# artpixls/ART

Hardware: AMD Instinct MI355X
Metric: megapixels/sec end-to-end (AMaZE+FTblockDN+tone), 45 MP Bayer (higher is better)
Workload: dtype f32; 1 GPU; AMaZE + getImage/matrix + ImProcFunctions::denoise (chroma noise-curve map, FTblockDN wavelet shrinkage luma 40 / chroma 15 / gamma 1.7 + DCT detail recovery 50) + exposure 0.3 EV + tone curve STD, 8192x5464 Bayer RGGB fp32, 1 frame per GPU per step (BASELINE configs[2]); frame=8192x5464, lanes_per_gpu=1, parallelism=frame-per-gpu x1, completion_records=1, completion_via=single process

## Files before the change

### art_amd/csrc/artgpu_api.hip

```cpp
#include <hip/hip_runtime.h>
#include <dlfcn.h>
#include <cmath>
#include <cstdio>
#include <cstdarg>
#include <cstring>
#include <new>
#include <string>
#include <thread>
#include <vector>
#include <algorithm>

#include "../../include/artgpu.h"
#include "kernels.h"
#include "dehaze.h"
#include "textureboost.h"
#include "colorcorrection.h"
#include "smoothing.h"
#include "masks.h"
#include "sharpen.h"

using namespace artgpu;

struct artgpu_ctx {
    int device = 0;
    hipStream_t stream = nullptr;
    hipStream_t aux = nullptr;
    hipEvent_t aux_ev[2] = {nullptr, nullptr};
    hipStream_t dn_stream[1] = {nullptr};
    hipEvent_t dn_ev[2] = {nullptr, nullptr};
    const float *gam_tab = nullptr; float gam_key[6] = {};
    struct Shared {
        int opt_sharpen_fused = 1;
        int opt_lut_lds = 1;
        int opt_dn_streams = 0;
        int opt_dn_fused = 1;
        int opt_dn_detail_plain = 0;
        int opt_dn_debug_stall = -1;
        long opt_dn_wait_ms = 0;
        int opt_io_direct = -1;
        int opt_amaze_path = 0;
        int opt_amaze_split = 0;
        long opt_amaze_zero_mask = 0x81f0;
        int opt_amaze_zero_frame = 16;
        int opt_amaze_poison = -1;
        int opt_roctx = 0;
        int opt_amaze_overlap = 1;
        int opt_amaze_grid = 0;
        int opt_rcd_rows = 8;
        int curve_tail_kind = ARTGPU_CURVE_TAIL_HOST;
        double curve_tail_y = 1.0;
        ParamCurve curve_tail_pc = {};
        artgpu_progress_fn progress_fn = nullptr;
        void *progress_user = nullptr;
        const artgpu_mask_params *pipe_lc = nullptr, *pipe_tb = nullptr;
        int pipe_nlc = 0, pipe_ntb = 0;
        const artgpu_color_correction_region *pipe_cc = nullptr;
        const artgpu_mask_params *pipe_cc_masks = nullptr;
        int pipe_ncc = 0;
        const artgpu_smoothing_region *pipe_sm = nullptr;
        const artgpu_mask_params *pipe_sm_masks = nullptr;
        int pipe_nsm = 0;
    } shared;
    float *sh_host = nullptr;
    hipEvent_t sh_ev = nullptr;
    struct PipeMasks { std::vector<artgpu_mask_params> m; std::vector<std::vector<double>> curves; std::vector<artgpu_plane> areas; } pipe_lc_own, pipe_tb_own;
    template <typename Region> struct PipeRegions { std::vector<Region> regs; std::vector<artgpu_plane> planes; PipeMasks masks; };
    PipeRegions<artgpu_color_correction_region> pipe_cc_own;
    PipeRegions<artgpu_smoothing_region> pipe_sm_own;
    std::string err;
    int *fs_diag = nullptr;
    long long batch_px = 0;
    int dn_form = -1, dn_form_streak = 0;
    float *arena = nullptr;
    size_t arena_bytes = 0;
    static constexpr int NSTAGE = 8;
    float *stage[NSTAGE] = {};
    size_t stage_bytes[NSTAGE] = {};
    static constexpr int NPOOL = 96;
    float *pool[NPOOL] = {};
    size_t pool_bytes[NPOOL] = {};
    std::vector<artgpu_ctx *> lanes;
    int batch_lanes = 1;
    int frames_in_flight = 1;
    bool owns_stream = false;
    hipStream_t io_up = nullptr, io_down = nullptr;
    hipEvent_t io_ev[8] = {};
    int *io_host = nullptr;
    int io_host_cap = 0;
    int cu_reserve = 0;
    float *bbox = nullptr;
    size_t bbox_bytes = 0;
    float *amz_lists = nullptr;
    size_t amz_lists_bytes = 0;
    int amz_w = 0, amz_h = 0, amz_nstream = 0, amz_narena = 0, amz_mode = -1;
    int num_cus = 0;
    hipStream_t amz_side = nullptr;
    hipEvent_t amz_ev[2] = {nullptr, nullptr};
    int *rcd_counter = nullptr;
    float *lut = nullptr;
    size_t lut_bytes = 0;
    std::vector<float> lut_host;
    std::vector<float> ncurve_host;
    char *tab_ring = nullptr;
    size_t tab_ring_bytes = 0, tab_ring_off = 0;
    bool tab_ring_busy = false;
    hipEvent_t tab_ev = nullptr;
    std::vector<float> rgbcurve_host[3];
    bool timing = false;
    hipEvent_t ev[3] = {nullptr, nullptr, nullptr};
    artgpu_timings last = {0.f, 0.f, 0.f};
};

namespace {

int fail(artgpu_ctx *ctx, int code, const char *fmt, ...)
{
    char buf[512];
    va_list ap;
    va_start(ap, fmt);
    vsnprintf(buf, sizeof buf, fmt, ap);
    va_end(ap);
    if (ctx) {
        ctx->err = buf;
        if (code == ARTGPU_EHIP && ctx->fs_diag && (unsigned)ctx->fs_diag[0] == 0xF5D1A600u) {
            char more[192];
            snprintf(more, sizeof more, " [shrink_blur_kernel: band %d strip %d gave up waiting for the strip above to hand down block %d (its counter: %d)]",
                     ctx->fs_diag[1], ctx->fs_diag[2], ctx->fs_diag[3], ctx->fs_diag[4]);
            ctx->err += more;
            ctx->fs_diag[0] = 0;
        }
    }
    return code;
}

#define HIPCHK(ctx, call)                                                                        \
    do {                                                                                         \
        hipError_t e_ = (call);                                                                  \
        if (e_ != hipSuccess)                                                                    \
            return fail(ctx, ARTGPU_EHIP, "%s failed: %s (%s:%d)", #call, hipGetErrorString(e_), __FILE__, __LINE__); \
    } while (0)

struct SideStreamJoin {
    hipStream_t side = nullptr;
    void arm(hipStream_t s) { side = s; }
    void disarm() { side = nullptr; }
    ~SideStreamJoin() { if (side) (void)hipStreamSynchronize(side); }
};

int ensure(artgpu_ctx *ctx, float **buf, size_t *cur, size_t need)
{
    if (*cur >= need) return ARTGPU_OK;
    if (*buf) { HIPCHK(ctx, hipFree(*buf)); *buf = nullptr; *cur = 0; }
    hipError_t e = hipMalloc(reinterpret_cast<void **>(buf), need);
    if (e != hipSuccess) {
        *buf = nullptr;
        return fail(ctx, ARTGPU_ENOMEM, "hipMalloc(%zu bytes) failed: %s", need, hipGetErrorString(e));
    }
    *cur = need;
    return ARTGPU_OK;
}

int h2d_table(artgpu_ctx *ctx, void *dst, const void *src, size_t bytes)
{
    const size_t need = (bytes + 255) & ~(size_t)255;
    if (need > ctx->tab_ring_bytes) {
        if (ctx->tab_ring) {
            if (ctx->tab_ring_busy) HIPCHK(ctx, hipEventSynchronize(ctx->tab_ev));
            HIPCHK(ctx, hipHostFree(ctx->tab_ring));
            ctx->tab_ring = nullptr; ctx->tab_ring_bytes = 0; ctx->tab_ring_busy = false;
        }
        const size_t cap = need * 2 > ((size_t)8 << 20) ? need * 2 : ((size_t)8 << 20);
        if (hipHostMalloc(reinterpret_cast<void **>(&ctx->tab_ring), cap, hipHostMallocDefault) != hipSuccess) {
            ctx->tab_ring = nullptr;
            return fail(ctx, ARTGPU_ENOMEM, "pinned staging ring for look-up tables (%zu bytes)", cap);
        }
        ctx->tab_ring_bytes = cap; ctx->tab_ring_off = 0;
        if (!ctx->tab_ev) HIPCHK(ctx, hipEventCreateWithFlags(&ctx->tab_ev, hipEventDisableTiming));
    }
    if (ctx->tab_ring_off + need > ctx->tab_ring_bytes) {
        if (ctx->tab_ring_busy) HIPCHK(ctx, hipEventSynchronize(ctx->tab_ev));
        ctx->tab_ring_busy = false;
        ctx->tab_ring_off = 0;
    }
    char *slot = ctx->tab_ring + ctx->tab_ring_off;
    std::memcpy(slot, src, bytes);
    HIPCHK(ctx, hipMemcpyAsync(dst, slot, bytes, hipMemcpyHostToDevice, ctx->stream));
    HIPCHK(ctx, hipEventRecord(ctx->tab_ev, ctx->stream));
    ctx->tab_ring_busy = true;
    ctx->tab_ring_off += need;
    return ARTGPU_OK;
}

bool plane_ok(const artgpu_plane *p)
{
    return p && p->p && p->w > 0 && p->h > 0 && p->row_stride_bytes >= (int64_t)p->w * 4 && (p->row_stride_bytes % 4) == 0;
}

struct DevImage {
    const float *raw; size_t raw_stride;
    float *r, *g, *b; size_t out_stride;
    bool staged;
};

int bind_images(artgpu_ctx *ctx, const artgpu_plane *raw, artgpu_rgb *out, DevImage *d)
{
    const int W = raw->w, H = raw->h;
    const artgpu_plane *op[3] = {&out->r, &out->g, &out->b};
    for (int k = 0; k < 3; ++k) {
        if (!plane_ok(op[k]) || op[k]->w != W || op[k]->h != H) return fail(ctx, ARTGPU_EINVAL, "output plane %d: bad pointer/size/stride", k);
        if ((op[k]->on_device != 0) != (out->r.on_device != 0) || op[k]->row_stride_bytes != out->r.row_stride_bytes)
            return fail(ctx, ARTGPU_EINVAL, "output planes must share residency and row stride");
    }
    d->staged = false;
    if (raw->on_device) {
        d->raw = raw->p;
        d->raw_stride = (size_t)(raw->row_stride_bytes / 4);
    } else {
        int rc = ensure(ctx, &ctx->stage[0], &ctx->stage_bytes[0], (size_t)W * H * 4);
        if (rc) return rc;
        HIPCHK(ctx, hipMemcpy2DAsync(ctx->stage[0], (size_t)W * 4, raw->p, (size_t)raw->row_stride_bytes, (size_t)W * 4, H, hipMemcpyHostToDevice, ctx->stream));
        d->raw = ctx->stage[0];
        d->raw_stride = W;
    }
    if (out->r.on_device) {
// ... 80 lines not shown
    d->staged = true;
    return ARTGPU_OK;
}

int unbind_rgb(artgpu_ctx *ctx, artgpu_rgb *img, const DevRGB *d)
{
    if (!d->staged) return ARTGPU_OK;
    artgpu_plane *pl[3] = {&img->r, &img->g, &img->b};
    const size_t rowb = (size_t)d->w * 4;
    for (int k = 0; k < 3; ++k)
        HIPCHK(ctx, hipMemcpy2DAsync(pl[k]->p, (size_t)pl[k]->row_stride_bytes, d->p[k], rowb, rowb, d->h, hipMemcpyDeviceToHost, ctx->stream));
    HIPCHK(ctx, hipStreamSynchronize(ctx->stream));
    return ARTGPU_OK;
}

#ifndef ARTGPU_MAX_TILE_WG
#define ARTGPU_MAX_TILE_WG 8192
#endif
constexpr int MAX_TILE_WORKGROUPS = ARTGPU_MAX_TILE_WG;

}

extern "C" {

const char *artgpu_version(void) { return "artgpu 0.1 (gfx950)"; }

int artgpu_create(int hip_device, artgpu_ctx **out)
{
    if (!out) return ARTGPU_EINVAL;
    *out = nullptr;
    int n = 0;
    if (hipGetDeviceCount(&n) != hipSuccess || n <= 0 || hip_device < 0 || hip_device >= n) return ARTGPU_EHIP;
    artgpu_ctx *ctx = new (std::nothrow) artgpu_ctx;
    if (!ctx) return ARTGPU_ENOMEM;
    ctx->device = hip_device;
    if (hipSetDevice(hip_device) != hipSuccess) { delete ctx; return ARTGPU_EHIP; }
    for (int k = 0; k < 3; ++k)
        if (hipEventCreate(&ctx->ev[k]) != hipSuccess) {
            for (int j = 0; j < k; ++j) (void)hipEventDestroy(ctx->ev[j]);
            delete ctx;
            return ARTGPU_EHIP;
        }
    *out = ctx;
    return ARTGPU_OK;
}

int artgpu_destroy(artgpu_ctx *ctx)
{
    if (!ctx) return ARTGPU_EINVAL;
    (void)hipSetDevice(ctx->device);
    (void)hipStreamSynchronize(ctx->stream);
    if (ctx->arena) (void)hipFree(ctx->arena);
    for (int k = 0; k < artgpu_ctx::NSTAGE; ++k)
        if (ctx->stage[k]) (void)hipFree(ctx->stage[k]);
    if (ctx->lut) (void)hipFree(ctx->lut);
    if (ctx->tab_ring) (void)hipHostFree(ctx->tab_ring);
    if (ctx->fs_diag) (void)hipHostFree(ctx->fs_diag);
    if (ctx->sh_host) (void)hipHostFree(ctx->sh_host);
    if (ctx->sh_ev) (void)hipEventDestroy(ctx->sh_ev);
    if (ctx->tab_ev) (void)hipEventDestroy(ctx->tab_ev);
    if (ctx->bbox) (void)hipFree(ctx->bbox);
    if (ctx->amz_lists) (void)hipFree(ctx->amz_lists);
    if (ctx->rcd_counter) (void)hipFree(ctx->rcd_counter);
    for (int k = 0; k < artgpu_ctx::NPOOL; ++k)
        if (ctx->pool[k]) (void)hipFree(ctx->pool[k]);
    for (int k = 0; k < 3; ++k)
        if (ctx->ev[k]) (void)hipEventDestroy(ctx->ev[k]);
    for (artgpu_ctx *l : ctx->lanes) (void)artgpu_destroy(l);
    ctx->lanes.clear();
    if (ctx->io_up) { (void)hipStreamSynchronize(ctx->io_up); (void)hipStreamDestroy(ctx->io_up); }
    if (ctx->io_down) { (void)hipStreamSynchronize(ctx->io_down); (void)hipStreamDestroy(ctx->io_down); }
    for (int k = 0; k < 8; ++k)
        if (ctx->io_ev[k]) (void)hipEventDestroy(ctx->io_ev[k]);
    if (ctx->io_host) (void)hipHostFree(ctx->io_host);
    if (ctx->owns_stream && ctx->stream) (void)hipStreamDestroy(ctx->stream);
    for (int k = 0; k < 2; ++k)
        if (ctx->aux_ev[k]) (void)hipEventDestroy(ctx->aux_ev[k]);
    if (ctx->aux) { (void)hipStreamSynchronize(ctx->aux); (void)hipStreamDestroy(ctx->aux); }
    for (int k = 0; k < 2; ++k)
        if (ctx->dn_ev[k]) (void)hipEventDestroy(ctx->dn_ev[k]);
    if (ctx->dn_stream[0]) { (void)hipStreamSynchronize(ctx->dn_stream[0]); (void)hipStreamDestroy(ctx->dn_stream[0]); }
    for (int k = 0; k < 2; ++k)
        if (ctx->amz_ev[k]) (void)hipEventDestroy(ctx->amz_ev[k]);
    if (ctx->amz_side) { (void)hipStreamSynchronize(ctx->amz_side); (void)hipStreamDestroy(ctx->amz_side); }
    delete ctx;
    return ARTGPU_OK;
}

const char *artgpu_last_error(const artgpu_ctx *ctx) { return ctx ? ctx->err.c_str() : "null context"; }

int artgpu_set_stream(artgpu_ctx *ctx, void *hip_stream)
{
    if (!ctx) return ARTGPU_EINVAL;
    hipStream_t next = static_cast<hipStream_t>(hip_stream);
    if (next == ctx->stream) return ARTGPU_OK;
    HIPCHK(ctx, hipSetDevice(ctx->device));
    hipEvent_t ev = nullptr;
    if (hipEventCreateWithFlags(&ev, hipEventDisableTiming) == hipSuccess) {
        if (hipEventRecord(ev, ctx->stream) == hipSuccess) (void)hipStreamWaitEvent(next, ev, 0);
        (void)hipEventDestroy(ev);
    }
    (void)hipGetLastError();
    ctx->stream = next;
    return ARTGPU_OK;
}

static int check_async_faults(artgpu_ctx *ctx)
{
    if (ctx->fs_diag && (unsigned)ctx->fs_diag[0] == 0xF5D1A600u) return fail(ctx, ARTGPU_EHIP, "a kernel gave up a bounded wait: the results of the calls since the last synchronisation are invalid");
    return ARTGPU_OK;
}

int artgpu_synchronize(artgpu_ctx *ctx)
{
    if (!ctx) return ARTGPU_EINVAL;
    HIPCHK(ctx, hipSetDevice(ctx->device));
    HIPCHK(ctx, hipStreamSynchronize(ctx->stream));
    return check_async_faults(ctx);
}

int artgpu_set_curve_tail(artgpu_ctx *ctx, int kind, double y_last)
{
    if (!ctx) return ARTGPU_EINVAL;
    if (kind < ARTGPU_CURVE_TAIL_LUT || kind > ARTGPU_CURVE_TAIL_HOST) return fail(ctx, ARTGPU_EINVAL, "set_curve_tail: kind %d (a parametric curve: artgpu_set_curve_tail_parametric)", kind);
    ctx->shared.curve_tail_kind = kind;
    ctx->shared.curve_tail_y = y_last;
    return ARTGPU_OK;
}

int artgpu_set_curve_tail_parametric(artgpu_ctx *ctx, const double *p, int np)
{
    if (!ctx) return ARTGPU_EINVAL;
    if (!p || (np != 8 && np != 9)) return fail(ctx, ARTGPU_EINVAL, "set_curve_tail_parametric: 8 or 9 parameters (p[0] = DCT_Parametric)");
    if (p[4] == 0.0 && p[5] == 0.0 && p[6] == 0.0 && p[7] == 0.0) return fail(ctx, ARTGPU_EINVAL, "set_curve_tail_parametric: an identity curve has no Curve object (ARTGPU_CURVE_TAIL_LUT)");
    pc_init(ctx->shared.curve_tail_pc, p, np);
    ctx->shared.curve_tail_kind = ARTGPU_CURVE_TAIL_PARAMETRIC;
    return ARTGPU_OK;
}

int artgpu_get_option(artgpu_ctx *ctx, const char *name, long *value)
{
    if (!ctx || !name || !value) return ARTGPU_EINVAL;
    const std::string n(name);
    if (n.rfind("amaze_counter", 0) == 0 && n.size() == 14 && n[13] >= '0' && n[13] <= '7') {
        if (!ctx->amz_lists || ctx->amz_nstream <= 0) { *value = 0; return ARTGPU_OK; }
        HIPCHK(ctx, hipSetDevice(ctx->device));
        HIPCHK(ctx, hipStreamSynchronize(ctx->stream));
        const size_t nfixed = (((size_t)ctx->amz_nstream + (1 + ctx->amz_narena) + (1 + ctx->amz_narena + ctx->amz_nstream) + 3) / 4) * 4;
        int v = 0;
        HIPCHK(ctx, hipMemcpy(&v, reinterpret_cast<int *>(ctx->amz_lists) + nfixed + 4 + 2 * (size_t)ctx->amz_nstream + (n[13] - '0'), sizeof(int), hipMemcpyDeviceToHost));
        *value = v;
        return ARTGPU_OK;
    }
    return fail(ctx, ARTGPU_EINVAL, "get_option: unknown option '%s'", name);
}

int artgpu_set_option(artgpu_ctx *ctx, const char *name, long value)
{
    if (!ctx || !name) return ARTGPU_EINVAL;
    const std::string n(name);
    if (n == "amaze_path") { if (value < 0 || value > 1) return fail(ctx, ARTGPU_EINVAL, "amaze_path: 0 or 1"); ctx->shared.opt_amaze_path = (int)value; }
    else if (n == "amaze_split") ctx->shared.opt_amaze_split = value != 0;
    else if (n == "amaze_overlap") ctx->shared.opt_amaze_overlap = value != 0;
    else if (n == "amaze_grid") { if (value < 0) return fail(ctx, ARTGPU_EINVAL, "amaze_grid: >= 0"); ctx->shared.opt_amaze_grid = (int)value; }
    else if (n == "amaze_zero_mask") ctx->shared.opt_amaze_zero_mask = value;
    else if (n == "amaze_zero_frame") ctx->shared.opt_amaze_zero_frame = (int)value;
    else if (n == "amaze_poison") ctx->shared.opt_amaze_poison = (int)value;
    else if (n == "roctx") ctx->shared.opt_roctx = value != 0;
    else if (n == "dn_streams") ctx->shared.opt_dn_streams = value != 0;
    else if (n == "dn_fused") ctx->shared.opt_dn_fused = (int)value;
    else if (n == "dn_detail_plain") { if (value < 0 || value > 3) return fail(ctx, ARTGPU_EINVAL, "dn_detail_plain: 0 .. 3"); ctx->shared.opt_dn_detail_plain = (int)value; }
    else if (n == "dn_debug_stall") ctx->shared.opt_dn_debug_stall = (int)value;
    else if (n == "dn_wait_ms") ctx->shared.opt_dn_wait_ms = value < 0 ? 0 : value;
    else if (n == "lut_lds") ctx->shared.opt_lut_lds = value != 0;
    else if (n == "sharpen_fused") ctx->shared.opt_sharpen_fused = value != 0;
    else if (n == "cu_reserve") { if (value < 0 || value > 4096) return fail(ctx, ARTGPU_EINVAL, "cu_reserve: 0 .. 4096"); ctx->cu_reserve = (int)value; }
    else if (n == "io_direct") { if (value < -1 || value > 4096) return fail(ctx, ARTGPU_EINVAL, "io_direct: -1 (automatic), 0 .. 4096 workgroups"); ctx->shared.opt_io_direct = (int)value; }
    else if (n == "rcd_rows") { if (value != 4 && value != 8) return fail(ctx, ARTGPU_EINVAL, "rcd_rows: 4 or 8"); ctx->shared.opt_rcd_rows = (int)value; }
    else return fail(ctx, ARTGPU_EINVAL, "set_option: unknown option '%s'", name);
    return ARTGPU_OK;
}

int artgpu_set_progress_callback(artgpu_ctx *ctx, artgpu_progress_fn fn, void *user)
{
    if (!ctx) return ARTGPU_EINVAL;
    ctx->shared.progress_fn = fn;
    ctx->shared.progress_user = user;
    return ARTGPU_OK;
}

int artgpu_enable_timing(artgpu_ctx *ctx, int enable)
{
    if (!ctx) return ARTGPU_EINVAL;
    ctx->timing = enable != 0;
    return ARTGPU_OK;
}

int artgpu_get_timings(const artgpu_ctx *ctx, artgpu_timings *out)
{
    if (!ctx || !out) return ARTGPU_EINVAL;
    *out = ctx->last;
    return ARTGPU_OK;
}

size_t artgpu_scratch_bytes(const artgpu_ctx *ctx)
{
    if (!ctx) return 0;
    size_t s = ctx->arena_bytes;
    for (int k = 0; k < artgpu_ctx::NSTAGE; ++k) s += ctx->stage_bytes[k];
    s += ctx->lut_bytes;
    for (int k = 0; k < artgpu_ctx::NPOOL; ++k) s += ctx->pool_bytes[k];
    return s;
}

int artgpu_trim_scratch(artgpu_ctx *ctx)
{
    if (!ctx) return ARTGPU_EINVAL;
    HIPCHK(ctx, hipSetDevice(ctx->device));
    HIPCHK(ctx, hipStreamSynchronize(ctx->stream));
    if (ctx->aux) HIPCHK(ctx, hipStreamSynchronize(ctx->aux));
    if (ctx->dn_stream[0]) HIPCHK(ctx, hipStreamSynchronize(ctx->dn_stream[0]));
    if (ctx->amz_side) HIPCHK(ctx, hipStreamSynchronize(ctx->amz_side));
    if (ctx->io_up) HIPCHK(ctx, hipStreamSynchronize(ctx->io_up));
    if (ctx->io_down) HIPCHK(ctx, hipStreamSynchronize(ctx->io_down));
    auto drop = [](float **p, size_t *b) { if (*p) (void)hipFree(*p); *p = nullptr; *b = 0; };
    drop(&ctx->arena, &ctx->arena_bytes);
    for (int k = 0; k < artgpu_ctx::NSTAGE; ++k) drop(&ctx->stage[k], &ctx->stage_bytes[k]);
    for (int k = 0; k < artgpu_ctx::NPOOL; ++k) drop(&ctx->pool[k], &ctx->pool_bytes[k]);
    ctx->batch_px = 0;
    ctx->gam_tab = nullptr;
    ctx->ncurve_host.clear();
    for (int k = 0; k < 3; ++k) ctx->rgbcurve_host[k].clear();
    int rc = ARTGPU_OK;
    for (artgpu_ctx *l : ctx->lanes) { const int r = artgpu_trim_scratch(l); if (r && !rc) rc = r; }
    return rc;
}

struct StageScope {
    artgpu_ctx *ctx;
    const char *name;
    bool range;
    typedef int (*push_fn)(const char *);
    typedef int (*pop_fn)();
    static push_fn &push() { static push_fn f = nullptr; return f; }
    static pop_fn &pop() { static pop_fn f = nullptr; return f; }
    StageScope(artgpu_ctx *c, const char *n) : ctx(c), name(n), range(false)
    {
        if (!ctx) return;
        if (ctx->shared.opt_roctx) {
            static bool tried = false;
            if (!tried) {
                tried = true;
                void *h = nullptr;
                for (const char *lib : {"libroctx64.so.4", "libroctx64.so", "/opt/rocm/lib/libroctx64.so"})
                    if ((h = dlopen(lib, RTLD_NOW | RTLD_GLOBAL))) break;
                if (h) {
                    push() = reinterpret_cast<push_fn>(dlsym(h, "roctxRangePushA"));
                    pop() = reinterpret_cast<pop_fn>(dlsym(h, "roctxRangePop"));
                }
            }
            if (push() && pop()) { push()(name); range = true; }
        }
        if (ctx->shared.progress_fn) ctx->shared.progress_fn(ctx->shared.progress_user, name, 0.0);
    }
    ~StageScope()
    {
        if (!ctx) return;
        if (ctx->shared.progress_fn) ctx->shared.progress_fn(ctx->shared.progress_user, name, 1.0);
        if (range) pop()();
    }
};

struct DualReq { double *contrast; int auto_contrast; int second; };
static int vng4_dev(artgpu_ctx *ctx, const float *raw, size_t raw_stride, float *r, float *g, float *b, size_t out_stride, int W, int H, uint32_t filters);
static int dual_blend_dev(artgpu_ctx *ctx, const DevImage &d, int W, int H, uint32_t filters, DualReq *req);
static int demosaic_bayer_impl(artgpu_ctx *ctx, int method, const artgpu_plane *raw, uint32_t filters,
                               double initial_gain, int border, artgpu_rgb *out, DualReq *dual)
{
    StageScope scope_(ctx, "RawImageSource::demosaic (Bayer)");
    if (!ctx) return ARTGPU_EINVAL;
    if (!plane_ok(raw) || !out) return fail(ctx, ARTGPU_EINVAL, "demosaic_bayer: bad raw plane or null output");
    if (method != ARTGPU_BAYER_AMAZE && method != ARTGPU_BAYER_RCD && method != ARTGPU_BAYER_VNG4) return fail(ctx, ARTGPU_EUNSUPPORTED, "demosaic_bayer: method %d is not on the device path", method);
    if (!(initial_gain > 0.0)) return fail(ctx, ARTGPU_EINVAL, "demosaic_bayer: initial_gain must be > 0");
    for (unsigned r = 0; r < 2; ++r)
        for (unsigned c = 0; c < 2; ++c)
            if (((filters >> ((((r << 1) & 14) + (c & 1)) << 1)) & 3) == 3) return fail(ctx, ARTGPU_EUNSUPPORTED, "demosaic_bayer: 4-colour CFA");
    const int W = raw->w, H = raw->h;
    if (W < 64 || H < 64) return fail(ctx, ARTGPU_EUNSUPPORTED, "demosaic_bayer: image %dx%d smaller than 64x64", W, H);
    HIPCHK(ctx, hipSetDevice(ctx->device));

    DevImage d;
    int rc = bind_images(ctx, raw, out, &d);
    if (rc) return rc;
    if (ctx->timing) HIPCHK(ctx, hipEventRecord(ctx->ev[0], ctx->stream));

    int bord = 0;
    if (method == ARTGPU_BAYER_AMAZE) {
        const int nty = (H + 16 + AMAZE_STEP - 1) / AMAZE_STEP, ntx = (W + 16 + AMAZE_STEP - 1) / AMAZE_STEP;
        const int ntiles = nty * ntx;
        const int mode = ctx->shared.opt_amaze_path;
        if (ctx->amz_w != W || ctx->amz_h != H || ctx->amz_mode != mode) {
            std::vector<int> st, ar;
            for (int ty = 0; ty < nty; ++ty)
                for (int tx = 0; tx < ntx; ++tx) {
                    const int top = -16 + ty * AMAZE_STEP, left = -16 + tx * AMAZE_STEP;
                    const int rr1 = std::min(top + AMAZE_TS, H + 16) - top, cc1 = std::min(left + AMAZE_TS, W + 16) - left;
                    if (rr1 <= 32 || cc1 <= 32) continue;
                    const bool wide = cc1 == AMAZE_TS && (left + AMAZE_TS <= W || left + AMAZE_TS == W + 16);
                    const bool rows_ok = rr1 < AMAZE_TS || top + AMAZE_TS <= H || top + AMAZE_TS == H + 16;
                    (mode == 0 && wide && rows_ok ? st : ar).push_back(ty * ntx + tx);
                }
            const size_t nfixed = ((st.size() + (1 + ar.size()) + (1 + ar.size() + st.size()) + 3) / 4) * 4;
            const size_t nints = nfixed + 4 + 2 * st.size() + 8;
            if ((rc = ensure(ctx, &ctx->amz_lists, &ctx->amz_lists_bytes, nints * sizeof(int)))) return rc;
            std::vector<int> hostbuf;
            hostbuf.insert(hostbuf.end(), st.begin(), st.end());
            hostbuf.push_back((int)ar.size());
            hostbuf.insert(hostbuf.end(), ar.begin(), ar.end());
            HIPCHK(ctx, hipMemcpyAsync(ctx->amz_lists, hostbuf.data(), hostbuf.size() * sizeof(int), hipMemcpyHostToDevice, ctx->stream));
            HIPCHK(ctx, hipStreamSynchronize(ctx->stream));
            ctx->amz_w = W; ctx->amz_h = H; ctx->amz_mode = mode;
            ctx->amz_nstream = (int)st.size(); ctx->amz_narena = (int)ar.size();
        }
        int *const d_stream = reinterpret_cast<int *>(ctx->amz_lists);
        int *const d_templ = d_stream + ctx->amz_nstream;
        int *const d_work = d_templ + 1 + ctx->amz_narena;
        const size_t nfixed = (((size_t)ctx->amz_nstream + (1 + ctx->amz_narena) + (1 + ctx->amz_narena + ctx->amz_nstream) + 3) / 4) * 4;
        int *const d_queue = d_stream + nfixed;
        unsigned long long *const d_qwords = reinterpret_cast<unsigned long long *>(d_queue + 4);
        const float clip_pt = (float)(1.0 / initial_gain);
        const float clip_pt8 = (float)(0.8 / initial_gain);
        const bool split = mode == 1 && ctx->shared.opt_amaze_split;
        const bool early = ctx->amz_nstream > 0 && ctx->amz_narena > 0 && ctx->shared.opt_amaze_overlap;
        const int nlist_max = ctx->amz_narena + ctx->amz_nstream;
        const int cap = split ? MAX_TILE_WORKGROUPS : 768;
        const int grid = split ? std::min(ntiles, cap) : std::max(1, std::min(nlist_max, cap));
        rc = ensure(ctx, &ctx->arena, &ctx->arena_bytes, (size_t)grid * AMAZE_ARENA_FLOATS * sizeof(float));
        if (rc) return rc;
        if ((rc = ensure(ctx, &ctx->bbox, &ctx->bbox_bytes, (size_t)grid * 4 * sizeof(int)))) return rc;
        AmazeArgs a;
        a.raw = d.raw; a.raw_stride = d.raw_stride;
        a.red = d.r; a.green = d.g; a.blue = d.b; a.out_stride = d.out_stride;
        a.arena = ctx->arena;
        a.W = W; a.H = H; a.ntx = ntx; a.ntiles = ntiles;
        a.filters = filters;
        a.clip_pt = clip_pt;
        a.clip_pt8 = clip_pt8;
        a.bbox = reinterpret_cast<int *>(ctx->bbox);
        a.zero_mask = (unsigned)ctx->shared.opt_amaze_zero_mask;
        a.zero_frame = ctx->shared.opt_amaze_zero_frame;
        a.split = split ? 1 : 0;
        a.queue_words = d_qwords;
        a.queue_counters = reinterpret_cast<int *>(d_qwords + ctx->amz_nstream);
        if (ctx->shared.opt_amaze_poison >= 0)
            HIPCHK(ctx, hipMemsetAsync(ctx->arena, ctx->shared.opt_amaze_poison, (size_t)grid * AMAZE_ARENA_FLOATS * sizeof(float), ctx->stream));
        HIPCHK(ctx, hipMemsetAsync(d_queue, 0, (4 + 2 * (size_t)ctx->amz_nstream + 8) * sizeof(int), ctx->stream));
        SideStreamJoin amz_join;
        if (early) {
            HIPCHK(ctx, hipMemsetAsync(d_work, 0, sizeof(int), ctx->stream));
            if (!ctx->amz_side) {
                HIPCHK(ctx, hipStreamCreateWithFlags(&ctx->amz_side, hipStreamNonBlocking));
                for (int k = 0; k < 2; ++k) HIPCHK(ctx, hipEventCreateWithFlags(&ctx->amz_ev[k], hipEventDisableTiming));
            }
            HIPCHK(ctx, hipEventRecord(ctx->amz_ev[0], ctx->stream));
            HIPCHK(ctx, hipStreamWaitEvent(ctx->amz_side, ctx->amz_ev[0], 0));
            amz_join.arm(ctx->amz_side);
            a.tile_list = d_templ + 1; a.tile_count = d_templ;
            a.queue_hdr = nullptr;
            HIPCHK(ctx, launch_amaze(a, std::min(ctx->amz_narena, cap), ctx->stream));
        } else {
            HIPCHK(ctx, hipMemcpyAsync(d_work, d_templ, (size_t)(1 + ctx->amz_narena) * sizeof(int), hipMemcpyDeviceToDevice, ctx->stream));
        }
        if (ctx->amz_nstream > 0) {
            AmazeStreamArgs sa;
            sa.raw = d.raw; sa.raw_stride = d.raw_stride;
            sa.red = d.r; sa.green = d.g; sa.blue = d.b; sa.out_stride = d.out_stride;
            sa.W = W; sa.H = H; sa.ntx = ntx;
            sa.filters = filters;
            sa.clip_pt = clip_pt; sa.clip_pt8 = clip_pt8;
            const unsigned f00 = (filters >> 0) & 3, f01 = (filters >> 2) & 3;
            sa.g00 = (int)(f00 & 1);
            sa.ey = f00 == 1 ? (f01 == 0 ? 0 : 1) : (f00 == 0 ? 0 : 1);
            sa.tiles = d_stream; sa.ntiles = ctx->amz_nstream;
// ... 224 lines not shown
namespace {
int wavelet_skip(int level) { return level <= 1 ? 1 : 1 << (level - 1); }
}

extern "C" {

int artgpu_wavelet_decompose(artgpu_ctx *ctx, const artgpu_plane *src, int maxlvl, artgpu_wavelet **out)
{
    if (!ctx) return ARTGPU_EINVAL;
    if (!plane_ok(src) || !out || maxlvl < 1 || maxlvl > 9) return fail(ctx, ARTGPU_EINVAL, "wavelet_decompose: bad arguments");
    *out = nullptr;
    const int w = src->w, h = src->h, w2 = (w + 1) / 2, h2 = (h + 1) / 2;
    if ((w2 < h2 ? w2 : h2) < 2 * wavelet_skip(maxlvl - 1) || w < 8 || h < 8)
        return fail(ctx, ARTGPU_EUNSUPPORTED, "wavelet_decompose: %dx%d too small for %d levels", w, h, maxlvl);
    HIPCHK(ctx, hipSetDevice(ctx->device));
    const float *dsrc = src->p;
    size_t sstride = (size_t)(src->row_stride_bytes / 4);
    if (!src->on_device) {
        int rc = ensure(ctx, &ctx->stage[0], &ctx->stage_bytes[0], (size_t)w * h * 4);
        if (rc) return rc;
        HIPCHK(ctx, hipMemcpy2DAsync(ctx->stage[0], (size_t)w * 4, src->p, (size_t)src->row_stride_bytes, (size_t)w * 4, h, hipMemcpyHostToDevice, ctx->stream));
        dsrc = ctx->stage[0];
        sstride = w;
    }
    artgpu_wavelet *wv = new (std::nothrow) artgpu_wavelet;
    if (!wv) return fail(ctx, ARTGPU_ENOMEM, "wavelet_decompose: out of host memory");
    wv->w = w; wv->h = h; wv->w2 = w2; wv->h2 = h2; wv->nlevels = maxlvl; wv->n = (size_t)w2 * h2;
    hipError_t e = hipMalloc(reinterpret_cast<void **>(&wv->bands), (size_t)maxlvl * 3 * wv->n * sizeof(float));
    if (e == hipSuccess) e = hipMalloc(reinterpret_cast<void **>(&wv->lowpass[0]), wv->n * sizeof(float));
    if (e == hipSuccess) e = hipMalloc(reinterpret_cast<void **>(&wv->lowpass[1]), wv->n * sizeof(float));
    if (e != hipSuccess) {
        artgpu_wavelet_free(ctx, wv);
        return fail(ctx, ARTGPU_ENOMEM, "wavelet_decompose: hipMalloc failed: %s", hipGetErrorString(e));
    }
    WaveArgs a = {};
    a.w = w; a.h = h; a.w2 = w2; a.h2 = h2;
    for (int l = 0; l < maxlvl; ++l) {
        a.b1 = wv->band(l, 1); a.b2 = wv->band(l, 2); a.b3 = wv->band(l, 3);
        hipError_t le;
        if (l == 0) {
            a.src = dsrc; a.src_stride = sstride; a.lo = wv->lowpass[0];
            wv->cur = 0;
            le = launch_wavelet_analysis0(a, ctx->stream);
        } else {
            a.src = wv->lowpass[wv->cur]; a.lo = wv->lowpass[wv->cur ^ 1]; a.skip = wavelet_skip(l);
            le = launch_wavelet_haar_analysis(a, ctx->stream);
            wv->cur ^= 1;
        }
        if (le != hipSuccess) {
            artgpu_wavelet_free(ctx, wv);
            return fail(ctx, ARTGPU_EHIP, "wavelet_decompose: launch failed: %s", hipGetErrorString(le));
        }
    }
    if (!src->on_device) {
        const hipError_t se = hipStreamSynchronize(ctx->stream);
        if (se != hipSuccess) {
            artgpu_wavelet_free(ctx, wv);
            return fail(ctx, ARTGPU_EHIP, "wavelet_decompose: %s", hipGetErrorString(se));
        }
    }
    *out = wv;
    return ARTGPU_OK;
}

int artgpu_wavelet_info(const artgpu_wavelet *wv, int32_t *w2, int32_t *h2, int32_t *nlevels)
{
    if (!wv) return ARTGPU_EINVAL;
    if (w2) *w2 = wv->w2;
    if (h2) *h2 = wv->h2;
    if (nlevels) *nlevels = wv->nlevels;
    return ARTGPU_OK;
}

int artgpu_wavelet_get_band(artgpu_ctx *ctx, const artgpu_wavelet *wv, int level, int dir, float *dst, int on_device)
{
    if (!ctx) return ARTGPU_EINVAL;
    if (!wv || !dst || dir < 0 || dir > 3 || (dir > 0 && (level < 0 || level >= wv->nlevels))) return fail(ctx, ARTGPU_EINVAL, "wavelet_get_band: bad arguments");
    HIPCHK(ctx, hipSetDevice(ctx->device));
    const float *p = dir == 0 ? wv->lowpass[wv->cur] : wv->band(level, dir);
    HIPCHK(ctx, hipMemcpyAsync(dst, p, wv->n * sizeof(float), on_device ? hipMemcpyDeviceToDevice : hipMemcpyDeviceToHost, ctx->stream));
    if (!on_device) HIPCHK(ctx, hipStreamSynchronize(ctx->stream));
    return ARTGPU_OK;
}

int artgpu_wavelet_set_band(artgpu_ctx *ctx, artgpu_wavelet *wv, int level, int dir, const float *src, int on_device)
{
    if (!ctx) return ARTGPU_EINVAL;
    if (!wv || !src || dir < 0 || dir > 3 || (dir > 0 && (level < 0 || level >= wv->nlevels))) return fail(ctx, ARTGPU_EINVAL, "wavelet_set_band: bad arguments");
    HIPCHK(ctx, hipSetDevice(ctx->device));
    float *p = dir == 0 ? wv->lowpass[wv->cur] : wv->band(level, dir);
    HIPCHK(ctx, hipMemcpyAsync(p, src, wv->n * sizeof(float), on_device ? hipMemcpyDeviceToDevice : hipMemcpyHostToDevice, ctx->stream));
    if (!on_device) HIPCHK(ctx, hipStreamSynchronize(ctx->stream));
    return ARTGPU_OK;
}

int artgpu_wavelet_reconstruct(artgpu_ctx *ctx, artgpu_wavelet *wv, artgpu_plane *dst, float blend)
{
    if (!ctx) return ARTGPU_EINVAL;
    if (!wv || !plane_ok(dst) || dst->w != wv->w || dst->h != wv->h) return fail(ctx, ARTGPU_EINVAL, "wavelet_reconstruct: bad arguments");
    HIPCHK(ctx, hipSetDevice(ctx->device));
    float *ddst = dst->p;
    size_t dstride = (size_t)(dst->row_stride_bytes / 4);
    if (!dst->on_device) {
        int rc = ensure(ctx, &ctx->stage[0], &ctx->stage_bytes[0], (size_t)wv->w * wv->h * 4);
        if (rc) return rc;
        HIPCHK(ctx, hipMemcpy2DAsync(ctx->stage[0], (size_t)wv->w * 4, dst->p, (size_t)dst->row_stride_bytes, (size_t)wv->w * 4, wv->h, hipMemcpyHostToDevice, ctx->stream));
        ddst = ctx->stage[0];
        dstride = wv->w;
    }
    WaveArgs a = {};
    a.w = wv->w; a.h = wv->h; a.w2 = wv->w2; a.h2 = wv->h2; a.blend = blend;
    for (int l = wv->nlevels - 1; l > 0; --l) {
        a.src = wv->lowpass[wv->cur]; a.lo = wv->lowpass[wv->cur ^ 1];
        a.b1 = wv->band(l, 1); a.b2 = wv->band(l, 2); a.b3 = wv->band(l, 3); a.skip = wavelet_skip(l);
        HIPCHK(ctx, launch_wavelet_haar_synthesis(a, ctx->stream));
        wv->cur ^= 1;
    }
    a.src = wv->lowpass[wv->cur];
    a.b1 = wv->band(0, 1); a.b2 = wv->band(0, 2); a.b3 = wv->band(0, 3);
    a.dst = ddst; a.dst_stride = dstride;
    HIPCHK(ctx, launch_wavelet_synthesis0(a, ctx->stream));
    if (!dst->on_device) {
        HIPCHK(ctx, hipMemcpy2DAsync(dst->p, (size_t)dst->row_stride_bytes, ddst, (size_t)wv->w * 4, (size_t)wv->w * 4, wv->h, hipMemcpyDeviceToHost, ctx->stream));
        HIPCHK(ctx, hipStreamSynchronize(ctx->stream));
    }
    return ARTGPU_OK;
}

int artgpu_wavelet_free(artgpu_ctx *ctx, artgpu_wavelet *wv)
{
    if (!wv) return ARTGPU_EINVAL;
    if (ctx) { (void)hipSetDevice(ctx->device); (void)hipStreamSynchronize(ctx->stream); }
    if (wv->bands) (void)hipFree(wv->bands);
    if (wv->lowpass[0]) (void)hipFree(wv->lowpass[0]);
    if (wv->lowpass[1]) (void)hipFree(wv->lowpass[1]);
    delete wv;
    return ARTGPU_OK;
}

}

namespace {

enum { P_L = 0, P_A, P_B, P_LBANDS, P_LLOW0, P_LLOW1, P_CBANDS, P_CLOW0, P_CLOW1, P_SF, P_TMP, P_HISTO, P_MAD, P_GAM, P_CCALC, P_LIN, P_BLOCKS, P_DTAB, P_CCMAP, P_CACHEF, P_PQ, P_XCBRT, P_GAUSS64, P_DMASK, P_LABTABS, P_PIPE_R, P_PIPE_G, P_PIPE_B, P_DNINFO, P_BATCH, P_DCTTAB, P_CBANDS2, P_CLOW0_2, P_CLOW1_2, P_SF_A, P_SF_B, P_HISTO_A, P_HISTO_B, P_RGBCURVES, P_FUSED, P_LBANDS2,
       P_IO_IN0, P_IO_IN1, P_IO_CFA, P_IO_IMG0, P_IO_IMG1, P_IO_IMG2, P_IO_IMG3, P_IO_IMG4, P_IO_IMG5, P_IO_OUT0, P_IO_OUT1, P_IO_FLAGS,
       P_CA_HALF, P_CA_BLK, P_CA_GUARD, P_CA_RAW,
       P_LC_BANDS, P_LC_LOW0, P_LC_LOW1, P_LC_NEW, P_LC_STATS, P_LC_MASK, P_LC_L,
       P_DH_STATE, P_DH_THUMB, P_DH_LOW, P_DH_TMP, P_DH_T, P_DH_DARK,
       P_SH_PLANES, P_SH_BYTES, P_SH_STATE,
       P_TB_PLANES, P_TB_LOW, P_TB_TMP, P_TB_STATE, P_TB_MASK, P_TB_Y,
       P_MK_WORK, P_MK_TAB, P_MK_CTHR, P_MK_AREA, P_MK_OUT,
       P_CC_MASK, P_CC_OOR, P_CC_GEN,
       P_SM_PLANES, P_SM_MASK, P_SM_BOX, P_SM_GEN,
       P_NSLOTS };
static_assert(P_NSLOTS <= artgpu_ctx::NPOOL, "grow artgpu_ctx::pool");

struct DevDecomp {
    float *bands, *low[2];
    int cur, nlevels, w, h, w2, h2;
    size_t n;
    float *band(int l, int dir) const { return bands + ((size_t)l * 3 + (dir - 1)) * n; }
};

int decompose_dev(artgpu_ctx *ctx, DevDecomp &d, const float *src, hipStream_t st = nullptr, size_t src_stride = 0)
{
    if (!st) st = ctx->stream;
    WaveArgs a = {};
    a.w = d.w; a.h = d.h; a.w2 = d.w2; a.h2 = d.h2;
    for (int l = 0; l < d.nlevels; ++l) {
        a.b1 = d.band(l, 1); a.b2 = d.band(l, 2); a.b3 = d.band(l, 3);
        if (l == 0) {
            a.src = src; a.src_stride = src_stride ? src_stride : (size_t)d.w; a.lo = d.low[0]; d.cur = 0;
            HIPCHK(ctx, launch_wavelet_analysis0(a, st));
        } else {
            a.src = d.low[d.cur]; a.lo = d.low[d.cur ^ 1]; a.skip = wavelet_skip(l);
            HIPCHK(ctx, launch_wavelet_haar_analysis(a, st));
            d.cur ^= 1;
        }
    }
    return ARTGPU_OK;
}

int reconstruct_dev(artgpu_ctx *ctx, DevDecomp &d, float *dst, hipStream_t st = nullptr)
{
    if (!st) st = ctx->stream;
    WaveArgs a = {};
    a.w = d.w; a.h = d.h; a.w2 = d.w2; a.h2 = d.h2; a.blend = 1.f;
    for (int l = d.nlevels - 1; l > 0; --l) {
        a.src = d.low[d.cur]; a.lo = d.low[d.cur ^ 1];
        a.b1 = d.band(l, 1); a.b2 = d.band(l, 2); a.b3 = d.band(l, 3); a.skip = wavelet_skip(l);
        HIPCHK(ctx, launch_wavelet_haar_synthesis(a, st));
        d.cur ^= 1;
    }
    a.src = d.low[d.cur];
    a.b1 = d.band(0, 1); a.b2 = d.band(0, 2); a.b3 = d.band(0, 3);
    a.dst = dst; a.dst_stride = d.w;
    HIPCHK(ctx, launch_wavelet_synthesis0(a, st));
    return ARTGPU_OK;
}

int pool_get(artgpu_ctx *ctx, int slot, size_t bytes, float **out)
{
    int rc = ensure(ctx, &ctx->pool[slot], &ctx->pool_bytes[slot], bytes);
    *out = ctx->pool[slot];
    return rc;
}

}

extern "C" {

namespace {
int detail_mask_dev(artgpu_ctx *ctx, const float *src, size_t src_stride, float *mask, int W, int H,
                    float scaling, float threshold, float ceiling, float factor, float blur, float *scratch);
}

int artgpu_wavelet_mad(artgpu_ctx *ctx, const artgpu_wavelet *wv, float *mad_sqr)
{
    if (!ctx) return ARTGPU_EINVAL;
    if (!wv || !mad_sqr) return fail(ctx, ARTGPU_EINVAL, "wavelet_mad: null argument");
    if (wv->n > 0x7fffffff) return fail(ctx, ARTGPU_EUNSUPPORTED, "wavelet_mad: band larger than an int holds (MadRgb's datalen is an int)");
    HIPCHK(ctx, hipSetDevice(ctx->device));
    const int nsub = 3 * wv->nlevels;
    float *histo_f, *mad;
    int rc;
    if ((rc = pool_get(ctx, P_HISTO, (size_t)nsub * (65536 + MAD_SCRATCH_INTS_PER_BAND) * 4, &histo_f)) || (rc = pool_get(ctx, P_MAD, 3 * 32 * 4, &mad))) return rc;
    HIPCHK(ctx, launch_mad(wv->bands, wv->n, nsub, reinterpret_cast<int *>(histo_f), mad, ctx->stream));
    HIPCHK(ctx, hipMemcpyAsync(mad_sqr, mad, (size_t)nsub * sizeof(float), hipMemcpyDeviceToHost, ctx->stream));
    HIPCHK(ctx, hipStreamSynchronize(ctx->stream));
    return ARTGPU_OK;
}

}

namespace {

struct DnFusion {
    float pre_scale, post_scale;
    GetImageFuse gi;
    int exp_on;
    float exp_scale, exp_black;
    int tail_on;
    float tail_scale, tail_black;
    int ccalc_nonneg;
};

int const_table_dev(artgpu_ctx *ctx, int slot, size_t nfloats, void (*fill)(float *), const char *what, float **out)
{
    const bool fresh = ctx->pool[slot] == nullptr;
    const int rc = pool_get(ctx, slot, nfloats * 4, out);
    if (rc || !fresh) return rc;
    std::vector<float> host(nfloats);
    fill(host.data());
    hipError_t e = hipMemcpyAsync(*out, host.data(), nfloats * 4, hipMemcpyHostToDevice, ctx->stream);
    if (e == hipSuccess) e = hipStreamSynchronize(ctx->stream);
    if (e != hipSuccess) {
        (void)hipFree(ctx->pool[slot]); ctx->pool[slot] = nullptr; ctx->pool_bytes[slot] = 0;
        *out = nullptr;
        return fail(ctx, ARTGPU_EHIP, "upload of the %s failed: %s", what, hipGetErrorString(e));
    }
    return ARTGPU_OK;
}

void build_lab_tabs(float *host)
{
    build_cachef(host); build_cachefy(host + 65536);
    build_denoise_gamma_tabs(host + 2 * 65536, host + 3 * 65536);
}

int lab_tabs_dev(artgpu_ctx *ctx, float **tabs_out)
{
    return const_table_dev(ctx, P_LABTABS, 4 * 65536, build_lab_tabs, "Lab tables", tabs_out);
}

void build_dct_tabs(float *host)
{
    float *tm_in = host, *tm_out = tm_in + 4096, *ct = tm_out + 4096, *ctt = ct + 4096;
    const float epsilon = 0.001f / (64 * 64);
    const int border = 4;
    for (int i = 0; i < 64; ++i) {
        const float i1 = std::abs((i > 32 ? i - 64 + 1 : i));
        const float vmask = (i1 < border ? (float)0 + (std::sin((M_PI * i1) / (2 * border)) * std::sin((M_PI * i1) / (2 * border))) : 1.0f);
        const float vmask2 = (i1 < 2 * border ? (std::sin((M_PI * i1) / (2 * border)) * std::sin((M_PI * i1) / (2 * border))) : 1.0f);
        for (int j = 0; j < 64; ++j) {
            const float j1 = std::abs((j > 32 ? j - 64 + 1 : j));
            const double sj = std::sin((M_PI * j1) / (2 * border));
            tm_in[i * 64 + j] = (vmask * (j1 < border ? sj * sj : 1.0f)) + epsilon;
            tm_out[i * 64 + j] = (vmask2 * (j1 < 2 * border ? sj * sj : 1.0f)) + epsilon;
            ct[i * 64 + j] = (float)std::cos(M_PI * (j + 0.5) * i / 64.0);
            ctt[j * 64 + i] = ct[i * 64 + j];
        }
    }
}

struct DnPlan {
    int w, h, w2, h2;
    size_t n, n2;
    bool lab_mode, do_detail, useNoiseCCurve;
    float noisevarL;
    bool denoiseLuminance;
    float gam, gamthresh, gamslope, igam, igamthresh, igamslope, gain;
    float realred, realblue, noisevarab_r, noisevarab_b, maxNoiseVarab;
    bool aggressive, autoch;
    int levwav, nsub;
    bool too_small;
    int rad[10], maxrad;
    bool fork;
    bool fused, merged, merged_mad;
    bool two_chroma;
    int detail_plain;
    long long wait_ticks;
    int stall_band, stall_strip;
};

DnPlan dn_plan(int w, int h, const artgpu_denoise_params *p, double scale, double expcomp, uint32_t flags, bool want_resid, bool has_ccalc,
               int opt_dn_streams, int opt_dn_fused, int opt_dn_detail_plain, long opt_dn_wait_ms, int opt_dn_debug_stall)
{
    DnPlan pl = {};
    const int w2 = (w + 1) / 2, h2 = (h + 1) / 2;
    pl.w = w; pl.h = h; pl.w2 = w2; pl.h2 = h2; pl.n = (size_t)w * h; pl.n2 = (size_t)w2 * h2;
    pl.lab_mode = p->color_space == 1;
    pl.do_detail = !(flags & ARTGPU_DN_SKIP_DETAIL_RECOVERY);
    pl.useNoiseCCurve = has_ccalc;
    pl.detail_plain = opt_dn_detail_plain == 1 ? 3 : opt_dn_detail_plain == 2 ? 1 : opt_dn_detail_plain == 3 ? 2 : 0;
    pl.wait_ticks = (long long)opt_dn_wait_ms * 100000LL;
    pl.stall_band = opt_dn_debug_stall < 0 ? -1 : opt_dn_debug_stall >> 16;
    pl.stall_strip = opt_dn_debug_stall < 0 ? -1 : opt_dn_debug_stall & 0xffff;

    const float noiseluma = (float)p->luminance;
    const double nl_t = (noiseluma / 125.0) * (1.0 + noiseluma / 25.0);
    const float noisevarL = (float)(nl_t * nl_t);
    const bool denoiseLuminance = noisevarL > 0.00001f;
    const float gam = (float)p->gamma;
    const float gamthresh = 0.001f;
    const float gamslope = (float)(std::exp(std::log((double)gamthresh) / gam) / gamthresh);
    pl.noisevarL = noisevarL; pl.denoiseLuminance = denoiseLuminance;
    pl.gam = gam; pl.gamthresh = gamthresh; pl.gamslope = gamslope;
    pl.igam = 1.f / gam; pl.igamthresh = gamthresh * gamslope; pl.igamslope = 1.f / gamslope;
    pl.gain = std::pow(2.0f, float(expcomp));
    const float interm_med = (float)p->chrominance / 10.0;
    float intermred = p->chrominance_red_green > 0. ? (p->chrominance_red_green / 10.) : (float)p->chrominance_red_green / 7.0;
    float intermblue = p->chrominance_blue_yellow > 0. ? (p->chrominance_blue_yellow / 10.) : (float)p->chrominance_blue_yellow / 7.0;
    float realred = interm_med + intermred;
    if (realred <= 0.f) realred = 0.001f;
    float realblue = interm_med + intermblue;
    if (realblue <= 0.f) realblue = 0.001f;
    const float noisevarab_r = realred * realred, noisevarab_b = realblue * realblue;
    pl.realred = realred; pl.realblue = realblue; pl.noisevarab_r = noisevarab_r; pl.noisevarab_b = noisevarab_b;
    pl.maxNoiseVarab = noisevarab_b > noisevarab_r ? noisevarab_b : noisevarab_r;
    int levwav = 5;
    const float maxreal = realred > realblue ? realred : realblue;
    if (maxreal < 8.f) levwav = 5; else if (maxreal < 10.f) levwav = 6; else if (maxreal < 15.f) levwav = 7; else levwav = 8;
    const bool aggressive = p->aggressive != 0;
    if (aggressive) levwav += 2;
    if (levwav > 8) levwav = 8;
    { const int t = int(levwav - std::ceil(std::log(scale))); levwav = t > 5 ? t : 5; }
    const int minsizetile = w < h ? w : h;
    int maxlev2 = 8;
    if (minsizetile < 256) maxlev2 = 7;
    if (minsizetile < 128) maxlev2 = 6;
    if (minsizetile < 64) maxlev2 = 5;
    if (minsizetile < 32) maxlev2 = 4;
    if (minsizetile < 16) maxlev2 = 3;
    levwav = levwav < maxlev2 ? levwav : maxlev2;
    const int nsub = 3 * levwav;
    const bool autoch = p->chrominance_method == 1;
    pl.aggressive = aggressive; pl.autoch = autoch; pl.levwav = levwav; pl.nsub = nsub;
    pl.too_small = (w2 < h2 ? w2 : h2) < 2 * wavelet_skip(levwav - 1) || w < 8 || h < 8;
    if (pl.too_small) return pl;

    pl.fork = opt_dn_streams != 0 && pl.do_detail && denoiseLuminance;

    pl.maxrad = 1;
    for (int l = 0; l < levwav; ++l) { const int r = int((l + 2) / scale); pl.rad[l] = r > 1 ? r : 1; pl.maxrad = pl.rad[l] > pl.maxrad ? pl.rad[l] : pl.maxrad; }
    pl.fused = opt_dn_fused != 0 && shrink_blur_supported(w2, h2, pl.rad, 0, nsub);
    pl.merged = pl.fused && opt_dn_fused != 2 && !aggressive && !want_resid && denoiseLuminance && levwav <= 5 &&
                (autoch || (noisevarab_r > 0.001f && noisevarab_b > 0.001f));
    pl.merged_mad = pl.merged && opt_dn_fused != 3;
    pl.two_chroma = pl.fork || pl.merged;
    return pl;
}

struct DnBuffers {
    float *L, *A, *B, *gamlut, *mad, *ccalc_dev;
    float *sfc[3], *tmpc[3], *histo_fc[3];
    DevDecomp Ld, Cdd[2];
    float *fused_scratch, *Lbands2;
};

int pool_drop(artgpu_ctx *ctx, int slot)
{
    if (!ctx->pool[slot]) return ARTGPU_OK;
    HIPCHK(ctx, hipStreamSynchronize(ctx->stream));
    if (ctx->dn_stream[0]) HIPCHK(ctx, hipStreamSynchronize(ctx->dn_stream[0]));
    HIPCHK(ctx, hipFree(ctx->pool[slot]));
    ctx->pool[slot] = nullptr; ctx->pool_bytes[slot] = 0;
    return ARTGPU_OK;
}

int dn_buffers(artgpu_ctx *ctx, const DnPlan &pl, const artgpu_plane *ccalc, DnBuffers *out)
{
    const int w2 = pl.w2, h2 = pl.h2, nsub = pl.nsub;
    const size_t n = pl.n, n2 = pl.n2;
    const bool fused = pl.fused, merged = pl.merged, merged_mad = pl.merged_mad;
    DnBuffers &b = *out;
    b = DnBuffers{};
    float *tmp1 = nullptr;
    DevDecomp &Ld = b.Ld, *Cdd = b.Cdd;
    Ld.w = pl.w; Ld.h = pl.h; Ld.w2 = w2; Ld.h2 = h2; Ld.n = n2; Ld.nlevels = pl.levwav;
    Cdd[0] = Cdd[1] = Ld;
    int rc;
    const size_t histo_bytes = (size_t)nsub * (65536 + MAD_SCRATCH_INTS_PER_BAND) * 4, band_bytes = (size_t)nsub * n2 * 4;
    if ((rc = pool_get(ctx, P_L, n * 4, &b.L)) || (rc = pool_get(ctx, P_A, n * 4, &b.A)) || (rc = pool_get(ctx, P_B, n * 4, &b.B)) ||
        (rc = pool_get(ctx, P_LBANDS, (merged_mad ? 3 : 1) * band_bytes, &Ld.bands)) || (rc = pool_get(ctx, P_LLOW0, n2 * 4, &Ld.low[0])) || (rc = pool_get(ctx, P_LLOW1, n2 * 4, &Ld.low[1])) ||
        (rc = merged_mad ? ARTGPU_OK : pool_get(ctx, P_CBANDS, (merged ? 2 : 1) * band_bytes, &Cdd[0].bands)) || (rc = pool_get(ctx, P_CLOW0, n2 * 4, &Cdd[0].low[0])) || (rc = pool_get(ctx, P_CLOW1, n2 * 4, &Cdd[0].low[1])) ||
        (rc = pool_get(ctx, P_HISTO, (merged_mad ? 3 : 1) * histo_bytes, &b.histo_fc[0])) ||
        (rc = pool_get(ctx, P_MAD, 3 * 32 * 4, &b.mad)) || (rc = pool_get(ctx, P_GAM, 2 * 65536 * 4, &b.gamlut)))
        return rc;
    if (ctx->dn_form == (fused ? 1 : 0)) ++ctx->dn_form_streak; else { ctx->dn_form = fused ? 1 : 0; ctx->dn_form_streak = 1; }
    const bool settle = ctx->dn_form_streak >= 4;
    if (fused) {
        if (settle && ((rc = pool_drop(ctx, P_SF_A)) || (rc = pool_drop(ctx, P_SF_B)) || (merged && (rc = pool_drop(ctx, P_CBANDS2))))) return rc;
        if (!ctx->fs_diag) {
            if (hipHostMalloc(reinterpret_cast<void **>(&ctx->fs_diag), 64, hipHostMallocDefault) == hipSuccess) std::memset(ctx->fs_diag, 0, 64);
            else { ctx->fs_diag = nullptr; (void)hipGetLastError(); }
        }
        if ((rc = pool_get(ctx, P_FUSED, shrink_blur_scratch_floats(w2, h2, merged ? 3 * nsub : nsub, pl.maxrad) * 4, &b.fused_scratch))) return rc;
        if ((pl.fork || merged) && (rc = pool_get(ctx, P_LBANDS2, band_bytes, &b.Lbands2))) return rc;
    } else if ((settle && ((rc = pool_drop(ctx, P_FUSED)) || (rc = pool_drop(ctx, P_LBANDS2)))) || (rc = pool_get(ctx, P_SF, band_bytes, &b.sfc[0])) || (rc = pool_get(ctx, P_TMP, band_bytes, &tmp1))) return rc;
    b.tmpc[0] = b.tmpc[1] = b.tmpc[2] = tmp1;
    if (pl.two_chroma) {
        if (merged_mad) Cdd[0].bands = Ld.bands + (size_t)nsub * n2;
        if (merged) Cdd[1].bands = Cdd[0].bands + (size_t)nsub * n2;
        else if ((rc = pool_get(ctx, P_CBANDS2, band_bytes, &Cdd[1].bands))) return rc;
        if ((rc = pool_get(ctx, P_CLOW0_2, n2 * 4, &Cdd[1].low[0])) || (rc = pool_get(ctx, P_CLOW1_2, n2 * 4, &Cdd[1].low[1])) ||
            (rc = pool_get(ctx, P_HISTO_A, (merged ? 2 : 1) * histo_bytes, &b.histo_fc[1])) || (rc = pool_get(ctx, P_HISTO_B, histo_bytes, &b.histo_fc[2])))
            return rc;
        if (!fused && ((rc = pool_get(ctx, P_SF_A, band_bytes, &b.sfc[1])) || (rc = pool_get(ctx, P_SF_B, band_bytes, &b.sfc[2])))) return rc;
    } else {
        b.sfc[1] = b.sfc[2] = b.sfc[0];
        b.histo_fc[1] = b.histo_fc[2] = b.histo_fc[0];
        Cdd[1] = Cdd[0];
    }
    if (pl.useNoiseCCurve) {
        if (!plane_ok(ccalc) || ccalc->w != w2 || ccalc->h != h2) return fail(ctx, ARTGPU_EINVAL, "rgb_denoise: ccalc must be %dx%d", w2, h2);
        if (ccalc->on_device && (size_t)ccalc->row_stride_bytes == (size_t)w2 * 4) {
            b.ccalc_dev = ccalc->p;
        } else {
            if ((rc = pool_get(ctx, P_CCALC, n2 * 4, &b.ccalc_dev))) return rc;
            HIPCHK(ctx, hipMemcpy2DAsync(b.ccalc_dev, (size_t)w2 * 4, ccalc->p, (size_t)ccalc->row_stride_bytes, (size_t)w2 * 4, h2,
                                         ccalc->on_device ? hipMemcpyDeviceToDevice : hipMemcpyHostToDevice, ctx->stream));
        }
    }
    return ARTGPU_OK;
}

struct DnRun {
    artgpu_ctx *ctx;
    const DnPlan &pl;
    DnBuffers &b;
    const DnFusion &fu;
    const artgpu_denoise_params *p;
    double scale;
    float *nresi, *highresi;
    hipStream_t sL;
    float noisevar_abc[2];
    float chresidtemp, chmaxresidtemp;
    float *Lout;

    BlurArgs blur0() const
    {
        BlurArgs bl0 = {};
        bl0.n = pl.n2; bl0.w = pl.w2; bl0.h = pl.h2;
        for (int l = 0; l < 10; ++l) bl0.rad[l] = pl.rad[l];
        return bl0;
    }
    FusedShrinkArgs fused_args(float nv_const) const
    {
        FusedShrinkArgs fa = {};
        fa.n = pl.n2; fa.w = pl.w2; fa.h = pl.h2;
        fa.noisevar = b.ccalc_dev; fa.noisevar_nonneg = fu.ccalc_nonneg; fa.noisevar_const = nv_const; fa.noisevar_scale = pl.maxNoiseVarab;
        fa.useNoiseCCurve = pl.useNoiseCCurve ? 1 : 0;
        for (int l = 0; l < 10; ++l) fa.rad[l] = pl.rad[l];
        fa.diag = ctx->fs_diag; fa.wait_ticks = pl.wait_ticks; fa.stall_band = pl.stall_band; fa.stall_strip = pl.stall_strip;
        return fa;
    }
    int fused_pass(bool ab, const float *cin, float *cout, const float *cL, const float *mL, const float *mab, int lev0, int nb, float nv_const, float noisevar_ab);
    int chroma_front(int ch);
    int chroma_back(int ch);
    int luma(hipStream_t sd);
    int detail_recovery(hipStream_t sd);
    int merged_pass();
};

int DnRun::fused_pass(bool ab, const float *cin, float *cout, const float *cL, const float *mL, const float *mab, int lev0, int nb,
                      float nv_const, float noisevar_ab)
{
    FusedShrinkArgs fa = fused_args(nv_const);
    if (ab) { fa.coefC = cout; fa.nL = 0; fa.nsub_ch = nb; }
    else { fa.coef = cin; fa.coef_out = cout; fa.nL = nb; }
    fa.coefL = cL;
    fa.madL = mL; fa.madab = mab;
    fa.noisevar_ab[0] = fa.noisevar_ab[1] = noisevar_ab;
    fa.level0 = lev0; fa.nsub = nb;
    HIPCHK(ctx, launch_shrink_blur(fa, b.fused_scratch, sL));
    return ARTGPU_OK;
}

int DnRun::chroma_front(int ch)
{
    const int nsub = pl.nsub;
    const size_t n2 = pl.n2;
    const DevDecomp &Ld = b.Ld;
    DevDecomp &Cd = b.Cdd[ch];
    float *sf = b.sfc[1 + ch], *tmp = b.tmpc[1 + ch], *madL = b.mad, *madab = b.mad + 32 * (1 + ch);
    int *histo = reinterpret_cast<int *>(b.histo_fc[1 + ch]);
    float noisevar_ab = ch == 0 ? pl.noisevarab_r : pl.noisevarab_b;
    if (pl.autoch && noisevar_ab <= 0.001f) noisevar_ab = 0.02f;
    noisevar_abc[ch] = noisevar_ab;
    int rc2;
    if ((rc2 = decompose_dev(ctx, Cd, ch == 0 ? b.A : b.B, sL))) return rc2;
    if (pl.aggressive && noisevar_ab > 0.001f) {
        HIPCHK(ctx, launch_mad(Cd.bands, n2, nsub, histo, madab, sL));
        ShrinkArgs sa = {};
        sa.n = n2; sa.noisevar = b.ccalc_dev; sa.noisevar_scale = pl.maxNoiseVarab; sa.noisevar_ab = noisevar_ab; sa.useNoiseCCurve = pl.useNoiseCCurve ? 1 : 0;
        const size_t top = (size_t)(nsub - 3) * n2;
        sa.coef = Cd.bands + top; sa.coefL = Ld.bands + top; sa.sfave = sf; sa.madL = madL + (nsub - 3); sa.madab = madab + (nsub - 3);
        if (pl.fused) {
            if ((rc2 = fused_pass(true, Cd.bands + top, Cd.bands + top, Ld.bands + top, madL + (nsub - 3), madab + (nsub - 3), pl.levwav - 1, 3, 0.f, noisevar_ab))) return rc2;
        } else {
            HIPCHK(ctx, launch_shrink_sf(sa, 3, true, sL));
            BlurArgs bt = blur0();
            bt.level0 = pl.levwav - 1;
            bt.src = sf; bt.dst = tmp;
            HIPCHK(ctx, launch_hblur(bt, 3, sL));
            bt.src = tmp; bt.sfave = sf; bt.coef = Cd.bands + top;
            HIPCHK(ctx, launch_vblur_combine(bt, 3, sL));
        }
        if (nsub > 3) {
            sa.coef = Cd.bands; sa.coefL = Ld.bands; sa.madL = madL; sa.madab = madab;
            HIPCHK(ctx, launch_bishrink_AB(sa, nsub - 3, sL));
        }
    }
    if (noisevar_ab > 0.001f && !pl.merged_mad) {
        HIPCHK(ctx, launch_mad(Cd.bands, n2, nsub, histo, ch == 1 && pl.merged ? b.mad + 32 + nsub : madab, sL));
        if (!pl.fused) {
            ShrinkArgs sa = {};
            sa.coef = Cd.bands; sa.coefL = Ld.bands; sa.sfave = sf; sa.n = n2; sa.madL = madL; sa.madab = madab;
            sa.noisevar = b.ccalc_dev; sa.noisevar_scale = pl.maxNoiseVarab; sa.noisevar_ab = noisevar_ab; sa.useNoiseCCurve = pl.useNoiseCCurve ? 1 : 0;
            HIPCHK(ctx, launch_shrink_sf(sa, nsub, true, sL));
        }
    }
    return ARTGPU_OK;
}

int DnRun::chroma_back(int ch)
{
    const int nsub = pl.nsub;
    DevDecomp &Cd = b.Cdd[ch];
    float *sf = b.sfc[1 + ch], *tmp = b.tmpc[1 + ch], *madab = b.mad + 32 * (1 + ch);
    int *histo = reinterpret_cast<int *>(b.histo_fc[1 + ch]);
    if (noisevar_abc[ch] > 0.001f && !pl.merged) {
        if (pl.fused) {
            int rc2 = fused_pass(true, Cd.bands, Cd.bands, b.Ld.bands, b.mad, madab, 0, nsub, 0.f, noisevar_abc[ch]);
            if (rc2) return rc2;
        } else {
            BlurArgs bl = blur0();
            bl.src = sf; bl.dst = tmp;
            HIPCHK(ctx, launch_hblur(bl, nsub, sL));
            bl.src = tmp; bl.sfave = sf; bl.coef = Cd.bands;
            HIPCHK(ctx, launch_vblur_combine(bl, nsub, sL));
        }
    }
    if (nresi || highresi) {
        float host[32];
        HIPCHK(ctx, launch_mad(Cd.bands, pl.n2, nsub, histo, madab, sL));
        HIPCHK(ctx, hipMemcpyAsync(host, madab, (size_t)nsub * sizeof(float), hipMemcpyDeviceToHost, sL));
        HIPCHK(ctx, hipStreamSynchronize(sL));
        float resid = 0.f, maxresid = 0.f;
        for (int k = 0; k < nsub; ++k) {
            resid += host[k];
            if (host[k] > maxresid) maxresid = host[k];
        }
        if (ch == 0) { chresidtemp = resid; chmaxresidtemp = maxresid; }
        else {
            float chresid = resid + chresidtemp, chmaxresid = maxresid + chmaxresidtemp;
            chresid = std::sqrt(chresid / (6 * (pl.levwav)));
            if (highresi) *highresi = chresid + 0.66f * (std::sqrt(chmaxresid) - chresid);
            if (nresi) *nresi = chresid;
        }
    }
    return reconstruct_dev(ctx, Cd, ch == 0 ? b.A : b.B, sL);
}

int DnRun::luma(hipStream_t sd)
{
    if (!pl.denoiseLuminance) return ARTGPU_OK;
    int rc2;
    const int nsub = pl.nsub, nsubL = 3 * (pl.levwav < 5 ? pl.levwav : 5);
    const size_t n2 = pl.n2;
    const DevDecomp &Ld = b.Ld;
    float *sf = b.sfc[0], *tmp = b.tmpc[0];
    BlurArgs bl = blur0();
    ShrinkArgs sa = {};
    sa.coef = Ld.bands; sa.sfave = sf; sa.n = n2; sa.madL = b.mad; sa.noisevar = nullptr; sa.noisevar_const = pl.noisevarL;
    DevDecomp Lrec = Ld;
    if (pl.merged) Lrec.bands = b.Lbands2;
    for (int rep = pl.aggressive ? 0 : 1; rep < 2 && !pl.merged; ++rep) {
        if (pl.fused) {
            float *dstb = b.Lbands2 ? b.Lbands2 : Ld.bands;
            if ((rc2 = fused_pass(false, Lrec.bands, dstb, nullptr, b.mad, nullptr, 0, nsubL, pl.noisevarL, 0.f))) return rc2;
            Lrec.bands = dstb;
        } else {
            HIPCHK(ctx, launch_shrink_sf(sa, nsubL, false, sL));
            bl.src = sf; bl.dst = tmp;
            HIPCHK(ctx, launch_hblur(bl, nsubL, sL));
            bl.src = tmp; bl.sfave = sf; bl.coef = Ld.bands;
            HIPCHK(ctx, launch_vblur_combine(bl, nsubL, sL));
        }
    }
    if (Lrec.bands != Ld.bands && nsubL < nsub)
        HIPCHK(ctx, hipMemcpyAsync(Lrec.bands + (size_t)nsubL * n2, Ld.bands + (size_t)nsubL * n2, (size_t)(nsub - nsubL) * n2 * 4, hipMemcpyDeviceToDevice, sL));
    if (pl.do_detail) {
        if ((rc2 = pool_get(ctx, P_LIN, pl.n * 4, &Lout))) return rc2;
    }
    Lrec.cur = Ld.cur;
    if ((rc2 = reconstruct_dev(ctx, Lrec, Lout, sL))) return rc2;
    return pl.do_detail ? detail_recovery(sd) : ARTGPU_OK;
}

int DnRun::detail_recovery(hipStream_t sd)
{
    const int w = pl.w, h = pl.h;
    int rc2;
    DetailArgs da = {};
    da.w = w; da.h = h;
    da.numblox_W = (int)std::ceil(((float)w) / 25) + 2;
    da.numblox_H = (int)std::ceil(((float)h) / 25) + 2;
    const float params_Ldetail = std::min(float(p->luminance_detail), 99.9f);
    auto compute_detail = [](float dd) -> float { const float t = static_cast<float>((100. - dd) * (100. - dd) + 50. * (100. - dd)) * 64 * 0.5f; return t * t; };
    da.detail_hi = compute_detail(params_Ldetail);
    da.detail_lo = compute_detail(0.f);
    { const int br = int(3 / scale); da.blur_rad = br > 1 ? br : 1; }
    float *dtab;
    if ((rc2 = const_table_dev(ctx, P_DCTTAB, 4 * 4096, build_dct_tabs, "DCT tables", &dtab))) return rc2;
    if ((rc2 = pool_get(ctx, P_BLOCKS, (size_t)da.numblox_W * da.numblox_H * 4096 * 4, &da.blocks))) return rc2;
    da.tm_in = dtab; da.tm_out = dtab + 4096; da.costab = dtab + 2 * 4096; da.costab_t = dtab + 3 * 4096;
    da.L = Lout; da.Lin = b.L;
    da.plain = pl.detail_plain;
    if (p->luminance_detail_threshold > 0) {
        float *dmask;
        if ((rc2 = pool_get(ctx, P_DMASK, pl.n * 4, &dmask))) return rc2;
        const float amount = std::max(0.f, std::min(float(p->luminance_detail_threshold) / 100.f, 1.f));
        float *dm_scratch = b.tmpc[0];
        if (!dm_scratch && (rc2 = pool_get(ctx, P_TMP, ((size_t)w * h + 2 * (size_t)(w / 4) * (h / 4)) * 4, &dm_scratch))) return rc2;
        if ((rc2 = detail_mask_dev(ctx, Lout, (size_t)w, dmask, w, h, 65535.f, 25.f, 10000.f, amount, (float)(25.f / scale), dm_scratch))) return rc2;
        da.mask = dmask; da.params_Ldetail = params_Ldetail;
    }
    if (sd != sL) {
        HIPCHK(ctx, hipEventRecord(ctx->dn_ev[0], sL));
        HIPCHK(ctx, hipStreamWaitEvent(sd, ctx->dn_ev[0], 0));
    }
    HIPCHK(ctx, launch_detail_blocks(da, sd));
    HIPCHK(ctx, launch_detail_gather(da, sd));
    if (sd != sL) HIPCHK(ctx, hipEventRecord(ctx->dn_ev[1], sd));
    return ARTGPU_OK;
}

int DnRun::merged_pass()
{
    const int nsub = pl.nsub;
    FusedShrinkArgs fa = fused_args(pl.noisevarL);
    fa.coef = b.Ld.bands; fa.coef_out = b.Lbands2; fa.coefC = b.Cdd[0].bands; fa.coefL = b.Ld.bands;
    fa.madL = b.mad; fa.madab = pl.merged_mad ? b.mad + nsub : b.mad + 32; fa.mad_ch_stride = nsub;
    fa.noisevar_ab[0] = noisevar_abc[0]; fa.noisevar_ab[1] = noisevar_abc[1];
    fa.level0 = 0; fa.nsub = 3 * nsub; fa.nL = nsub; fa.nsub_ch = nsub;
    HIPCHK(ctx, launch_shrink_blur(fa, b.fused_scratch, sL));
    return ARTGPU_OK;
}

int rgb_denoise_args_ok(artgpu_ctx *ctx, const artgpu_denoise_params *p, const float *iws, double scale)
{
    if (p->color_space != 0 && p->color_space != 1) return fail(ctx, ARTGPU_EINVAL, "rgb_denoise: color_space must be 0 (RGB) or 1 (LAB)");
    if (p->color_space == 1 && !iws) return fail(ctx, ARTGPU_EINVAL, "rgb_denoise: LAB mode needs the inverse working-space matrix");
    if (p->chrominance_method != 0 && p->chrominance_method != 1) return fail(ctx, ARTGPU_EINVAL, "rgb_denoise: chrominance_method must be 0 (MANUAL) or 1 (AUTOMATIC)");
    if (!(scale >= 1.0)) return fail(ctx, ARTGPU_EINVAL, "rgb_denoise: scale must be >= 1");
    return ARTGPU_OK;
}

int rgb_denoise_dev(artgpu_ctx *ctx, const DevRGB &d, const artgpu_denoise_params *p, const float ws[9], const float *iws,
                    double expcomp, double scale, const artgpu_plane *ccalc, uint32_t flags, float *nresi, float *highresi, const DnFusion &fu)
{
    const int w = d.w, h = d.h;
    if (w > 32767 || h > 32767) return fail(ctx, ARTGPU_EUNSUPPORTED, "rgb_denoise: the reference holds the size in short (FTblockDN.cc:1779)");
    if (p->luminance == 0 && p->chrominance == 0 && !ccalc) return ARTGPU_OK;
    const DnPlan pl = dn_plan(w, h, p, scale, expcomp, flags, nresi || highresi, ccalc != nullptr,
                              ctx->shared.opt_dn_streams, ctx->shared.opt_dn_fused, ctx->shared.opt_dn_detail_plain, ctx->shared.opt_dn_wait_ms, ctx->shared.opt_dn_debug_stall);
    if (pl.too_small) return fail(ctx, ARTGPU_EUNSUPPORTED, "rgb_denoise: %dx%d too small for %d wavelet levels on the device path", w, h, pl.levwav);
    DnBuffers b;
    int rc = dn_buffers(ctx, pl, ccalc, &b);
    if (rc) return rc;
    if (pl.fork && !ctx->dn_stream[0]) {
        HIPCHK(ctx, hipStreamCreateWithFlags(&ctx->dn_stream[0], hipStreamNonBlocking));
        for (int k = 0; k < 2; ++k) HIPCHK(ctx, hipEventCreateWithFlags(&ctx->dn_ev[k], hipEventDisableTiming));
    }
    hipStream_t sL = ctx->stream;

    {
        const float key[6] = {pl.gam, pl.gamthresh, pl.gamslope, pl.igam, pl.igamthresh, pl.igamslope};
        if (ctx->gam_tab != b.gamlut || std::memcmp(ctx->gam_key, key, sizeof key) != 0) {
            ctx->gam_tab = nullptr;
            HIPCHK(ctx, launch_gamma_lut(b.gamlut, pl.gam, pl.gamthresh, pl.gamslope, 65535.f, 65535.f, sL));
            HIPCHK(ctx, launch_gamma_lut(b.gamlut + 65536, pl.igam, pl.igamthresh, pl.igamslope, 65535.f, 65535.f, sL));
            std::memcpy(ctx->gam_key, key, sizeof key);
            ctx->gam_tab = b.gamlut;
        }
    }

    DnPixArgs px = {};
    for (int k = 0; k < 3; ++k) { px.rgb[k] = d.p[k]; px.ws1[k] = ws[3 + k]; }
    px.stride = d.stride; px.L = b.L; px.A = b.A; px.B = b.B; px.w = w; px.h = h;
    px.gain = pl.gain; px.newGain = 1.f / pl.gain;
    px.gam = pl.gam; px.gamthresh = pl.gamthresh; px.gamslope = pl.gamslope; px.igam = pl.igam; px.igamthresh = pl.igamthresh; px.igamslope = pl.igamslope;
    px.gamcurve = b.gamlut; px.igamcurve = b.gamlut + 65536;
    px.pre_scale = fu.pre_scale; px.post_scale = fu.post_scale; px.no_lds_lut = !ctx->shared.opt_lut_lds; px.cu_reserve = ctx->cu_reserve;
    px.gi = fu.gi; px.exp_on = fu.exp_on; px.exp_scale = fu.exp_scale; px.exp_black = fu.exp_black;
    px.igam_lds_lo = 8000;
    if (pl.lab_mode) {
        float *tabs;
        if ((rc = lab_tabs_dev(ctx, &tabs))) return rc;
        px.lab_mode = 1;
        px.cachef = tabs; px.cachefy = tabs + 65536; px.dn_gamma = tabs + 2 * 65536; px.dn_igamma = tabs + 3 * 65536;
        for (int k = 0; k < 9; ++k) { px.wpi[k] = ws[k]; px.iws[k] = iws[k]; }
    }
    px.realred = pl.realred; px.realblue = pl.realblue; px.qhighFactor = pl.aggressive ? 1.f / static_cast<float>(0.9) : 1.0f;
    HIPCHK(ctx, launch_rgb2yuv(px, sL));

    if ((rc = decompose_dev(ctx, b.Ld, b.L, sL))) return rc;
    if (!pl.merged_mad) HIPCHK(ctx, launch_mad(b.Ld.bands, pl.n2, pl.nsub, reinterpret_cast<int *>(b.histo_fc[0]), b.mad, sL));

    DnRun run = {ctx, pl, b, fu, p, scale, nresi, highresi, sL, {0.f, 0.f}, 0.f, 0.f, b.L};
    if (pl.merged) {
        if ((rc = run.chroma_front(0)) || (rc = run.chroma_front(1))) return rc;
        if (pl.merged_mad) HIPCHK(ctx, launch_mad(b.Ld.bands, pl.n2, 3 * pl.nsub, reinterpret_cast<int *>(b.histo_fc[0]), b.mad, sL));
        if ((rc = run.merged_pass())) return rc;
        SideStreamJoin dn_join;
        if (pl.fork) dn_join.arm(ctx->dn_stream[0]);
        if ((rc = run.luma(pl.fork ? ctx->dn_stream[0] : sL))) return rc;
        if ((rc = run.chroma_back(0)) || (rc = run.chroma_back(1))) return rc;
        if (pl.fork) {
            HIPCHK(ctx, hipStreamWaitEvent(sL, ctx->dn_ev[1], 0));
            dn_join.disarm();
        }
    } else if (!pl.fork) {
        for (int ch = 0; ch < 2; ++ch)
            if ((rc = run.chroma_front(ch)) || (rc = run.chroma_back(ch))) return rc;
        if ((rc = run.luma(sL))) return rc;
    } else {
        if ((rc = run.chroma_front(0)) || (rc = run.chroma_front(1))) return rc;
        SideStreamJoin dn_join;
        dn_join.arm(ctx->dn_stream[0]);
        if ((rc = run.luma(ctx->dn_stream[0]))) return rc;
        if ((rc = run.chroma_back(0)) || (rc = run.chroma_back(1))) return rc;
        HIPCHK(ctx, hipStreamWaitEvent(sL, ctx->dn_ev[1], 0));
        dn_join.disarm();
    }
    px.L = run.Lout;

    HIPCHK(ctx, launch_yuv2rgb(px, ctx->stream));
    return ARTGPU_OK;
}

}

extern "C" {

int artgpu_rgb_denoise(artgpu_ctx *ctx, artgpu_rgb *img, const artgpu_denoise_params *p, const float ws[9], const float *iws,
                       double expcomp, double scale, const artgpu_plane *ccalc, uint32_t flags,
                       float *nresi, float *highresi)
{
    StageScope scope_(ctx, "denoise::RGB_denoise");
    if (!ctx) return ARTGPU_EINVAL;
    if (!img || !p || !ws) return fail(ctx, ARTGPU_EINVAL, "rgb_denoise: null argument");
    int rc = rgb_denoise_args_ok(ctx, p, iws, scale);
    if (rc) return rc;
    HIPCHK(ctx, hipSetDevice(ctx->device));
    DevRGB d;
    if ((rc = bind_rgb(ctx, img, 4, true, &d, "rgb_denoise"))) return rc;
    if ((rc = rgb_denoise_dev(ctx, d, p, ws, iws, expcomp, scale, ccalc, flags, nresi, highresi, DnFusion{}))) return rc;
    return unbind_rgb(ctx, img, &d);
}

namespace {
int gf_subsampling(int w, int h, int r)
{
    if (r == 1) return 1;
    if ((w > h ? w : h) <= 600) return 1;
    for (int s = 5; s > 0; --s)
        if (r % s == 0) return s;
    const int t = r / 2;
    return t < 2 ? 2 : (t > 4 ? 4 : t);
}
}

int artgpu_denoise_guided_smoothing(artgpu_ctx *ctx, artgpu_rgb *img, const double ws[9], int guided_chroma_radius, double scale)
{
    StageScope scope_(ctx, "denoise::denoiseGuidedSmoothing");
    if (!ctx) return ARTGPU_EINVAL;
    if (!img || !ws || !(scale >= 1.0)) return fail(ctx, ARTGPU_EINVAL, "denoise_guided_smoothing: bad arguments");
    if (guided_chroma_radius == 0) return ARTGPU_OK;
    HIPCHK(ctx, hipSetDevice(ctx->device));
    DevRGB d;
    int rc = bind_rgb(ctx, img, 4, true, &d, "denoise_guided_smoothing");
    if (rc) return rc;
    const int W = d.w, H = d.h;
    int r = (int)std::round(guided_chroma_radius / scale);
    r = r > 0 ? r : 0;
    GuidedArgs g = {};
    for (int k = 0; k < 3; ++k) { g.rgb[k] = d.p[k]; g.ws1[k] = ws[3 + k]; }
    g.stride = d.stride; g.W = W; g.H = H; g.epsilon = 0.001f;
    const int sub = gf_subsampling(W, H, r);
    g.w = W / sub; g.h = H / sub;
    if (r == 0 || g.w < 8 || g.h < 8) return fail(ctx, ARTGPU_EUNSUPPORTED, "denoise_guided_smoothing: radius/scale combination not on the device path");
    const size_t n = (size_t)W * H, nl = (size_t)g.w * g.h;
    float *big, *low, *tmp;
    if ((rc = pool_get(ctx, P_SF, 7 * n * 4, &big)) || (rc = pool_get(ctx, P_TMP, 8 * nl * 4, &low)) || (rc = pool_get(ctx, P_LIN, 8 * nl * 4, &tmp))) return rc;
    for (int k = 0; k < 3; ++k) { g.in[k] = big + k * n; g.chan[k] = big + (3 + k) * n; }
    g.guide = big + 6 * n;
    for (int k = 0; k < 8; ++k) g.low[k] = low + k * nl;
    HIPCHK(ctx, launch_gf_prepare(g, ctx->stream));
    HIPCHK(ctx, launch_gf_subsample(g, ctx->stream));
    const float r1 = float(r) / sub;
    int rad = (int)r1;
    { const int hi = ((g.w < g.h ? g.w : g.h) - 1) / 2 - 1; rad = rad < hi ? rad : hi; rad = rad > 0 ? rad : 0; }
    BlurArgs bl = {};
    bl.n = nl; bl.w = g.w; bl.h = g.h; bl.steady_div = 1; bl.plain = 1;
    for (int l = 0; l < 10; ++l) bl.rad[l] = rad;
    auto blur_planes = [&](float *planes, int count) -> int {
        if (rad == 0) return ARTGPU_OK;
        bl.src = planes; bl.dst = tmp;
        HIPCHK(ctx, launch_hblur(bl, count, ctx->stream));
        bl.src = tmp; bl.dst = planes; bl.sfave = nullptr; bl.coef = nullptr;
        HIPCHK(ctx, launch_vblur_combine(bl, count, ctx->stream));
        return ARTGPU_OK;
    };
    if ((rc = blur_planes(low, 8))) return rc;
    HIPCHK(ctx, launch_gf_ab(g, ctx->stream));
    if ((rc = blur_planes(low + 2 * nl, 6))) return rc;
    HIPCHK(ctx, launch_gf_finish(g, ctx->stream));
    return unbind_rgb(ctx, img, &d);
}

static int guided_filter_dev(artgpu_ctx *ctx, const float *guide, const float *src, float *q, size_t q_stride, int W, int H, int r, float epsilon, int subsampling,
                             const char *who)
{
    const int sub = subsampling > 0 ? subsampling : gf_subsampling(W, H, r);
    GuidedArgs g = {};
    g.W = W; g.H = H; g.w = W / sub; g.h = H / sub; g.epsilon = epsilon; g.nch = 1;
    if (g.w < 1 || g.h < 1) return fail(ctx, ARTGPU_EINVAL, "%s: subsampling %d leaves no pixels", who, sub);
    const size_t nl = (size_t)g.w * g.h;
    float *low, *tmp;
    int rc;
    if ((rc = pool_get(ctx, P_TMP, 8 * nl * 4, &low)) || (rc = pool_get(ctx, P_LIN, 8 * nl * 4, &tmp))) return rc;
    g.guide = const_cast<float *>(guide); g.chan[0] = const_cast<float *>(src); g.q = q; g.q_stride = q_stride;
    for (int k = 0; k < 8; ++k) g.low[k] = low + k * nl;
    const float r1 = float(r) / sub;
    int rad = (int)r1;
    { const int hi = ((g.w < g.h ? g.w : g.h) - 1) / 2 - 1; rad = rad < hi ? rad : hi; rad = rad > 0 ? rad : 0; }
    if (rad > HBLUR_MAX_RADIUS) return fail(ctx, ARTGPU_EUNSUPPORTED, "%s: box radius %d (r / subsampling) is above the %d the blur kernels hold in LDS", who, rad, HBLUR_MAX_RADIUS);
    HIPCHK(ctx, launch_gf_subsample(g, ctx->stream));
    BlurArgs bl = {};
    bl.n = nl; bl.w = g.w; bl.h = g.h; bl.steady_div = 1; bl.plain = 1;
    for (int l = 0; l < 10; ++l) bl.rad[l] = rad;
    auto blur_plane = [&](float *plane) -> int {
        if (rad == 0) return ARTGPU_OK;
        bl.src = plane; bl.dst = tmp;
        HIPCHK(ctx, launch_hblur(bl, 1, ctx->stream));
        bl.src = tmp; bl.dst = plane; bl.sfave = nullptr; bl.coef = nullptr;
        HIPCHK(ctx, launch_vblur_combine(bl, 1, ctx->stream));
        return ARTGPU_OK;
    };
    if ((rc = blur_plane(g.low[0])) || (rc = blur_plane(g.low[1])) || (rc = blur_plane(g.low[2])) || (rc = blur_plane(g.low[5]))) return rc;
    HIPCHK(ctx, launch_gf_ab(g, ctx->stream));
    if ((rc = blur_plane(g.low[2])) || (rc = blur_plane(g.low[5]))) return rc;
    HIPCHK(ctx, launch_gf_finish_plain(g, ctx->stream));
    return ARTGPU_OK;
}

int artgpu_guided_filter(artgpu_ctx *ctx, const artgpu_plane *guide, const artgpu_plane *src, artgpu_plane *dst, int r, float epsilon, int subsampling)
{
    if (!ctx) return ARTGPU_EINVAL;
    if (!guide || !src || !dst || !plane_ok(guide) || !plane_ok(src) || !plane_ok(dst)) return fail(ctx, ARTGPU_EINVAL, "guided_filter: bad plane");
    const int W = src->w, H = src->h;
    if (guide->w != W || guide->h != H || dst->w != W || dst->h != H || r < 0) return fail(ctx, ARTGPU_EINVAL, "guided_filter: size mismatch / negative radius");
    HIPCHK(ctx, hipSetDevice(ctx->device));
    const size_t n = (size_t)W * H;
    float *big;
// ... 3287 lines not shown
```

### art_amd/csrc/denoise.hip

```cpp
#include <hip/hip_runtime.h>
#include "devmath.h"
#include "devsleef.h"
#include "labdev.h"
#include "kernels.h"

namespace artgpu {

__global__ void __launch_bounds__(256) gamma_lut_kernel(float *lut, float gamma, float start, float slope, float divisor, float factor)
{
    const int i = blockIdx.x * 256 + threadIdx.x;
    if (i >= 65536) return;
    const float gammav = 1.f / gamma;
    const float slopev = (slope / divisor) * factor;
    const float divisorv = xlogf_s(divisor);
    const float comparev = start * divisor;
    const int border = (int)(start * divisor);
    const int border1 = border - (border & 3), border2 = border1 + 4;
    const float iv = (float)i;
    float r;
    if (i < border1) {
        r = iv * slopev;
    } else if (i < border2) {
        const float r0 = iv * slopev;
        const float r1 = xexpf_v((xlogf_v(iv) - divisorv) * gammav) * factor;
// ... 239 lines not shown
        for (int k = 0; k < U; ++k) {
            const size_t i = (chunk0 + k * cstride) * 256 + threadIdx.x;
            if (i < n) {
                const int v = (int)fminf(fabsf(x[k]), 65535.f);
                atomicAdd(&h[v < MAD_SAMPLE_BINS ? v : MAD_SAMPLE_BINS], 1);
            }
        }
    }
    __syncthreads();
    for (int i = threadIdx.x; i <= MAD_SAMPLE_BINS; i += 256)
        if (h[i]) atomicAdd(&s[MAD_SAMPLE_OFF + i], h[i]);
}
__global__ void __launch_bounds__(256) mad_pick_kernel(int *scr)
{
    __shared__ int part[256];
    int *s = scr + (size_t)blockIdx.x * MAD_WIN_STRIDE;
    const int *h = s + MAD_SAMPLE_OFF;
    constexpr int PER = MAD_SAMPLE_BINS / 256;
    int p = 0;
    for (int i = 0; i < PER; ++i) p += h[threadIdx.x * PER + i];
    part[threadIdx.x] = p;
    __syncthreads();
    if (threadIdx.x == 0) {
        int total = h[MAD_SAMPLE_BINS];
        for (int i = 0; i < 256; ++i) total += part[i];
        const int half = total / 2, d = 3 * (int)sqrtf((float)total) + 1;
        auto first_reaching = [&](int target) {
            int count = 0, chunk = 0;
            while (chunk < 256 && count + part[chunk] < target) { count += part[chunk]; ++chunk; }
            if (chunk == 256) return -1;
            int b = chunk * PER;
            for (; b < (chunk + 1) * PER; ++b) { count += h[b]; if (count >= target) break; }
            return b;
        };
        int L = -1, Wn = 0;
        if (total > 0) {
            const int lo = half - d <= 0 ? 0 : first_reaching(half - d), hi = first_reaching(half + d);
            if (lo >= 0 && hi >= 0) {
                L = lo > 0 ? lo - 1 : 0;
                Wn = hi + 2 - L;
                Wn = Wn < MAD_REG_BINS ? MAD_REG_BINS : Wn;
                if (Wn > MAD_WMAX) L = -1;
            }
        }
        s[0] = 0; s[1] = L; s[2] = 0; s[3] = total; s[4] = Wn;
    }
}
#ifndef MAD_WINDOW_LOADS
#define MAD_WINDOW_LOADS 8
#endif
__global__ void __launch_bounds__(256) mad_window_kernel(const float *bands, size_t n, int *scr)
{
    __shared__ int win[MAD_WMAX];
    __shared__ int red[MAD_REG_BINS + 1];
    const int sub = blockIdx.y;
    int *s = scr + (size_t)sub * MAD_WIN_STRIDE;
    const int L = s[1], Wn = s[4];
    if (L < 0) return;
    const float *data = bands + (size_t)sub * n;
    for (int i = threadIdx.x; i < Wn; i += 256) win[i] = 0;
    if (threadIdx.x <= MAD_REG_BINS) red[threadIdx.x] = 0;
    __syncthreads();
    constexpr int U = MAD_WINDOW_LOADS;
    static_assert(U * 16 < 256, "the packed byte counters are flushed every 16 iterations");
    const size_t stride = (size_t)gridDim.x * 256;
    int below = 0, cnt[MAD_REG_BINS];
    unsigned long long packed = 0;
#pragma unroll
    for (int b = 0; b < MAD_REG_BINS; ++b) cnt[b] = 0;
    auto flush = [&]() {
#pragma unroll
        for (int b = 0; b < MAD_REG_BINS; ++b) cnt[b] += (int)((packed >> (8 * b)) & 0xffull);
        packed = 0;
    };
    int it = 0;
    for (size_t i0 = blockIdx.x * (size_t)256 + threadIdx.x; i0 < n; i0 += stride * U, ++it) {
        float x[U];
#pragma unroll
        for (int k = 0; k < U; ++k) { const size_t i = i0 + k * stride; x[k] = data[i < n ? i : n - 1]; }
#pragma unroll
        for (int k = 0; k < U; ++k) {
            int w = (int)fminf(fabsf(x[k]), 65535.f) - L;
            w = i0 + k * stride < n ? w : 0x10000;
            below += w < 0;
            packed += (unsigned)w < (unsigned)MAD_REG_BINS ? 1ull << (8 * w) : 0ull;
            if (w >= MAD_REG_BINS && w < Wn) atomicAdd(&win[w], 1);
        }
        if ((it & 15) == 15) flush();
    }
    flush();
#pragma unroll
    for (int o = 32; o > 0; o >>= 1) {
        below += __shfl_down(below, o);
#pragma unroll
        for (int b = 0; b < MAD_REG_BINS; ++b) cnt[b] += __shfl_down(cnt[b], o);
    }
    if ((threadIdx.x & 63) == 0) {
        atomicAdd(&red[MAD_REG_BINS], below);
#pragma unroll
        for (int b = 0; b < MAD_REG_BINS; ++b) atomicAdd(&red[b], cnt[b]);
    }
    __syncthreads();
    if (threadIdx.x < MAD_REG_BINS && red[threadIdx.x]) atomicAdd(&s[8 + threadIdx.x], red[threadIdx.x]);
    if (threadIdx.x == MAD_REG_BINS && red[MAD_REG_BINS]) atomicAdd(&s[2], red[MAD_REG_BINS]);
    for (int i = MAD_REG_BINS + threadIdx.x; i < Wn; i += 256)
        if (win[i]) atomicAdd(&s[8 + i], win[i]);
}
__global__ void __launch_bounds__(64) mad_window_finish_kernel(int *scr, int datalen, float *out)
{
    if (threadIdx.x) return;
    int *s = scr + (size_t)blockIdx.x * MAD_WIN_STRIDE;
    if (datalen <= 1) { out[blockIdx.x] = 0.f; s[0] = 1; return; }
    const int L = s[1], Wn = s[4], half = datalen / 2;
    int count = s[2];
    if (L < 0 || count >= half) return;
    for (int b = 0; b < Wn; ++b) {
        const int hb = s[8 + b];
        count += hb;
        if (count >= half) {
            const int median = L + b + 1, count_ = count - hb;
            const float q = ((median - 1) + (half - count_) / ((float)(count - count_)));
            const float r = (float)((double)q / 0.6745);
            out[blockIdx.x] = r * r;
            s[0] = 1;
            return;
        }
    }
}

__global__ void __launch_bounds__(256) mad_finish_kernel(const int *histo, int datalen, float *out, const int *done)
{
    __shared__ int part[256];
    const int sub = blockIdx.x;
    if (done && done[sub * MAD_WIN_STRIDE]) return;
    const int *h = histo + (size_t)sub * 65536;
    int s = 0;
    for (int i = 0; i < 256; ++i) s += h[threadIdx.x * 256 + i];
    part[threadIdx.x] = s;
    __syncthreads();
    if (threadIdx.x == 0) {
        float r = 0.f;
        if (datalen > 1) {
            const int half = datalen / 2;
            int count = 0, chunk = 0;
            while (chunk < 256 && count + part[chunk] < half) { count += part[chunk]; ++chunk; }
            int median = chunk * 256;
            while (count < half) { count += h[median]; ++median; }
            const int count_ = count - h[median - 1];
            const float q = ((median - 1) + (half - count_) / ((float)(count - count_)));
            r = (float)((double)q / 0.6745);
        }
        out[sub] = r * r;
    }
}

__global__ void __launch_bounds__(256) shrink_sf_L_kernel(ShrinkArgs a)
{
    const int sub = blockIdx.y, level = sub / 3;
    const float *c = a.coef + (size_t)sub * a.n;
    float *sf = a.sfave + (size_t)sub * a.n;
    const float mad_L = a.madL[sub];
    const float levelFactor = mad_L * 5.f / (float)(level + 1);
    const float eps = 0.01f;
    const size_t nv4 = (a.n / 4) * 4;
    constexpr int U = 4;
    const size_t stride = (size_t)gridDim.x * 256;
    for (size_t i0 = blockIdx.x * (size_t)256 + threadIdx.x; i0 < a.n; i0 += stride * U) {
        float cv[U], nvv[U];
#pragma unroll
        for (int k = 0; k < U; ++k) {
            const size_t i = i0 + k * stride, ic = i < a.n ? i : a.n - 1;
            cv[k] = c[ic];
            nvv[k] = a.noisevar ? a.noisevar[ic] : a.noisevar_const;
        }
#pragma unroll
        for (int k = 0; k < U; ++k) {
            const size_t i = i0 + k * stride;
            const float nv = nvv[k];
            const float mag = sqr(cv[k]);
            float r;
            if (i < nv4) {
                const float madv = nv * levelFactor;
                r = mag / (mag + madv * xexpf_v(-mag / (9.0f * madv)) + eps);
            } else {
                r = mag / (mag + levelFactor * nv * xexpf_s(-mag / (9 * levelFactor * nv)) + eps);
            }
            if (i < a.n) sf[i] = r;
        }
    }
}

__global__ void __launch_bounds__(256) shrink_sf_AB_kernel(ShrinkArgs a)
{
    const int sub = blockIdx.y;
    const float *c = a.coef + (size_t)sub * a.n;
    const float *cL = a.coefL + (size_t)sub * a.n;
    float *sf = a.sfave + (size_t)sub * a.n;
    const float mad_L = a.madL[sub];
    float madab = a.madab[sub];
    madab = a.useNoiseCCurve ? madab : madab * a.noisevar_ab;
    const float rmadLm9 = 1.f / (mad_L * 9.f);
    const size_t nv4 = (a.n / 4) * 4;
    constexpr int U = 4;
    const size_t stride = (size_t)gridDim.x * 256;
    for (size_t i0 = blockIdx.x * (size_t)256 + threadIdx.x; i0 < a.n; i0 += stride * U) {
        float cv[U], clv[U], nvv[U];
#pragma unroll
        for (int k = 0; k < U; ++k) {
            const size_t i = i0 + k * stride, ic = i < a.n ? i : a.n - 1;
            cv[k] = c[ic];
            clv[k] = cL[ic];
            nvv[k] = a.noisevar ? a.noisevar[ic] : 0.f;
        }
#pragma unroll
        for (int k = 0; k < U; ++k) {
            const size_t i = i0 + k * stride;
            const float nvc = a.noisevar ? a.noisevar_scale * nvv[k] : 1.f;
            const float mag_ab = sqr(cv[k]);
            float r;
            if (i < nv4) {
                const float mad_abv = nvc * madab;
                const float mag_L = sqr(clv[k]) * rmadLm9;
                r = 1.f - xexpf_v(-(mag_ab / mad_abv) - mag_L);
            } else {
                const float mag_L = sqr(clv[k]);
                r = 1.f - xexpf_s(-(mag_ab / (nvc * madab)) - (mag_L / (9.f * mad_L)));
            }
            if (i < a.n) sf[i] = r;
        }
    }
}

__global__ void __launch_bounds__(256) bishrink_AB_kernel(ShrinkArgs a)
{
    const int sub = blockIdx.y;
    float *c = a.coef + (size_t)sub * a.n;
    const float *cL = a.coefL + (size_t)sub * a.n;
    const float mad_Lr = a.madL[sub];
    const float mab = a.madab[sub];
    const float mad_abr = a.useNoiseCCurve ? a.noisevar_ab * mab : sqr(a.noisevar_ab) * mab;
    const float rmad_Lm9 = 1.f / (mad_Lr * 9.f);
    const size_t nv4 = (a.n / 4) * 4;
    for (size_t i = blockIdx.x * (size_t)256 + threadIdx.x; i < a.n; i += (size_t)gridDim.x * 256) {
        const float nvc = a.noisevar ? a.noisevar_scale * a.noisevar[i] : 1.f;
        const float tempab = c[i];
        const float mag_ab = sqr(tempab);
        if (i < nv4) {
            const float mad_abv = nvc * mad_abr;
            const float mag_L = sqr(cL[i]) * rmad_Lm9;
            c[i] = tempab * sqr(1.f - xexpf_v(-(mag_ab / mad_abv) - (mag_L)));
        } else {
            const float mag_L = sqr(cL[i]);
            c[i] = tempab * sqr(1.f - xexpf_s(-(mag_ab / (nvc * mad_abr)) - (mag_L / (9.f * mad_Lr))));
        }
    }
}

constexpr int HB_ROWS = 16, HB_COLS = 64;
template <int HB_MAXR, bool SDIV>
__global__ void __launch_bounds__(64) hblur_kernel(BlurArgs a)
{
    constexpr int HB_TW = HB_COLS + 2 * HB_MAXR + 2;
    __shared__ float sT[HB_ROWS][HB_TW + 1];
    __shared__ float oT[HB_ROWS][HB_COLS + 1];
    const int sub = blockIdx.y, level = a.level0 + sub / 3;
    const int rad = a.rad[level];
    const int W = a.w, H = a.h;
    const float *src = a.src + (size_t)sub * a.n;
    float *dst = a.dst + (size_t)sub * a.n;
    const int r0 = blockIdx.x * HB_ROWS;
    const int lane = threadIdx.x;
    const int myrow = r0 + lane;
    const int nrows = min(HB_ROWS, H - r0);
    float tempval = 0.f;
    int len = rad + 1;
    float reclen = 0.f;
    auto wave_lds_sync = []() {
        __builtin_amdgcn_fence(__ATOMIC_SEQ_CST, "wavefront");
        __builtin_amdgcn_wave_barrier();
    };
    {
        const int wc0 = -rad - 1, wn = HB_COLS + 2 * rad + 1;
        const int colA = wc0 + lane, colB = wc0 + lane + 64, colC = wc0 + lane + 128;
        const bool okA = colA >= 0 && colA < W, okB = (lane + 64 < wn) && colB >= 0 && colB < W;
        const bool okC = HB_MAXR > 31 && (lane + 128 < wn) && colC >= 0 && colC < W;
        for (int k0 = 0; k0 < HB_ROWS; k0 += 8) {
            float va[8], vb[8], vc[8];
#pragma unroll
            for (int i = 0; i < 8; ++i) {
                const int k = k0 + i;
                const size_t ro = (size_t)(r0 + k) * W;
                va[i] = (okA && k < nrows) ? src[ro + colA] : 0.f;
                vb[i] = (okB && k < nrows) ? src[ro + colB] : 0.f;
                if constexpr (HB_MAXR > 31) vc[i] = (okC && k < nrows) ? src[ro + colC] : 0.f;
            }
#pragma unroll
            for (int i = 0; i < 8; ++i) {
                sT[k0 + i][lane] = va[i];
                if (lane + 64 < wn) sT[k0 + i][lane + 64] = vb[i];
                if constexpr (HB_MAXR > 31) { if (lane + 128 < wn) sT[k0 + i][lane + 128] = vc[i]; }
            }
        }
    }
    wave_lds_sync();
    for (int c0 = 0; c0 < W; c0 += HB_COLS) {
        const bool more = c0 + HB_COLS < W;
// ... 128 lines not shown
            for (int x = lane; x < cend; x += 64) dst[(size_t)(r0 + k) * W + c0 + x] = oT[k * OS_ + x];
        __syncthreads();
    }
}

template <bool PLAIN>
__global__ void __launch_bounds__(64) vblur_combine_kernel(BlurArgs a)
{
    const int sub = blockIdx.y, level = a.level0 + sub / 3;
    const int rad = a.rad[level];
    const int W = a.w, H = a.h;
    const float *t = a.src + (size_t)sub * a.n;
    const float *sfave = a.sfave + (size_t)sub * a.n;
    float *coef = a.coef + (size_t)sub * a.n;
    const int col = blockIdx.x * 64 + threadIdx.x;
    if (col >= W) return;
    const size_t nv4 = (a.n / 4) * 4;
    const float eps = 0.01f;
    const bool vec = PLAIN ? true : col < (W / 4) * 4;
    float *plain_dst = PLAIN ? a.dst + (size_t)sub * a.n : nullptr;
    float tv = 0.f;
    float lenf = (float)(rad + 1);
    int leni = rad + 1;
    float rlen = 0.f;
    auto commit = [&](int row, float sfd, float sf, float c) {
        const size_t i = (size_t)row * W + col;
        if (plain_dst) { plain_dst[i] = sfd; return; }
        const float num = sqr(sfd) + sqr(sf), den = sfd + sf + eps;
        coef[i] = i < nv4 ? c * num / den : c * (num / den);
    };
    int row = 0;
    for (; row <= rad && row < H; ++row) {
        if (row == 0) {
            if (vec) {
                tv = t[col];
                for (int i = 1; i <= rad; i++) tv = tv + t[(size_t)i * W + col];
                tv = tv / lenf;
            } else {
                tv = t[col] / leni;
                for (int i = 1; i <= rad; i++) tv += t[(size_t)i * W + col] / leni;
            }
        } else if (vec) {
            const float lenp1 = lenf + 1.f;
            tv = (tv * lenf + t[(size_t)(row + rad) * W + col]) / lenp1;
            lenf = lenp1;
        } else {
            tv = (tv * leni + t[(size_t)(row + rad) * W + col]) / (leni + 1);
            leni++;
        }
        const size_t i = (size_t)row * W + col;
        commit(row, tv, PLAIN ? 0.f : sfave[i], PLAIN ? 0.f : coef[i]);
    }
    rlen = 1.f / lenf;
    const int steady_end = H - rad;
    constexpr int VB = PLAIN ? 24 : 8;
    float hi[VB], lo[VB], sf[VB], c[VB], nhi[VB], nlo[VB], nsf[VB], nc[VB];
    auto fetch = [&](int r, float *h_, float *l_, float *s_, float *c_) {
#pragma unroll
        for (int k = 0; k < VB; ++k) {
            h_[k] = t[(size_t)(r + k + rad) * W + col];
            l_[k] = t[(size_t)(r + k - rad - 1) * W + col];
            s_[k] = PLAIN ? 0.f : sfave[(size_t)(r + k) * W + col];
            c_[k] = PLAIN ? 0.f : coef[(size_t)(r + k) * W + col];
        }
    };
    if (row + VB <= steady_end) fetch(row, hi, lo, sf, c);
    for (; row + VB <= steady_end; row += VB) {
        const bool more = row + 2 * VB <= steady_end;
        fetch(more ? row + VB : row, nhi, nlo, nsf, nc);
#pragma unroll
        for (int k = 0; k < VB; ++k) {
            const float d = hi[k] - lo[k];
            tv = vec ? tv + d * rlen : tv + d / leni;
            commit(row + k, tv, sf[k], c[k]);
        }
#pragma unroll
        for (int k = 0; k < VB; ++k) { hi[k] = nhi[k]; lo[k] = nlo[k]; sf[k] = nsf[k]; c[k] = nc[k]; }
    }
    for (; row < steady_end; ++row) {
        const float d = t[(size_t)(row + rad) * W + col] - t[(size_t)(row - rad - 1) * W + col];
        tv = vec ? tv + d * rlen : tv + d / leni;
        const size_t i = (size_t)row * W + col;
        commit(row, tv, PLAIN ? 0.f : sfave[i], PLAIN ? 0.f : coef[i]);
    }
    for (; row < H; ++row) {
        if (vec) {
            const float lenm1 = lenf - 1.f;
            tv = (tv * lenf - t[(size_t)(row - rad - 1) * W + col]) / lenm1;
            lenf = lenm1;
        } else {
            tv = (tv * leni - t[(size_t)(row - rad - 1) * W + col]) / (leni - 1);
            leni--;
        }
        const size_t i = (size_t)row * W + col;
        commit(row, tv, PLAIN ? 0.f : sfave[i], PLAIN ? 0.f : coef[i]);
    }
}

static int flat_grid(long long n, int cap) { long long g = (n + 255) / 256; return (int)(g < cap ? g : cap); }

hipError_t launch_gamma_lut(float *lut, float gamma, float start, float slope, float divisor, float factor, hipStream_t s)
{
    hipLaunchKernelGGL(gamma_lut_kernel, dim3(256), dim3(256), 0, s, lut, gamma, start, slope, divisor, factor);
    return hipGetLastError();
}
static bool dn_lds_shape(const DnPixArgs &a, const float *lut, int *cus)
{
    if (a.lab_mode || !(a.gam > 1.f) || (long long)a.w * a.h < (1 << 22) || (reinterpret_cast<uintptr_t>(lut) & 15) || a.no_lds_lut || !device_block_fits(LUT_LDS_N * (int)sizeof(float), 1024)) return false;
    int dev = 0;
    *cus = 256;
    if (hipGetDevice(&dev) == hipSuccess) (void)hipDeviceGetAttribute(cus, hipDeviceAttributeMultiprocessorCount, dev);
    if (a.cu_reserve > 0) *cus = *cus - a.cu_reserve > 1 ? *cus - a.cu_reserve : 1;
    return true;
}
hipError_t launch_rgb2yuv(const DnPixArgs &a, hipStream_t s)
{
    int cus;
    if (dn_lds_shape(a, a.gamcurve, &cus)) {
        const size_t lds = (size_t)LUT_LDS_N * sizeof(float);
        hipError_t e = hipFuncSetAttribute(reinterpret_cast<const void *>(rgb2yuv_lds_kernel), hipFuncAttributeMaxDynamicSharedMemorySize, (int)lds);
        if (e != hipSuccess) return e;
        hipLaunchKernelGGL(rgb2yuv_lds_kernel, dim3(cus < a.h ? cus : a.h), dim3(1024), lds, s, a);
        return hipGetLastError();
    }
    hipLaunchKernelGGL(rgb2yuv_kernel, image_grid(a.w, a.h), dim3(256), 0, s, a);
    return hipGetLastError();
}
hipError_t launch_yuv2rgb(const DnPixArgs &a, hipStream_t s)
{
    int cus;
    if (dn_lds_shape(a, a.igamcurve, &cus)) {
        const size_t lds = (size_t)LUT_LDS_N * sizeof(float);
        hipError_t e = hipFuncSetAttribute(reinterpret_cast<const void *>(yuv2rgb_lds_kernel), hipFuncAttributeMaxDynamicSharedMemorySize, (int)lds);
        if (e != hipSuccess) return e;
        hipLaunchKernelGGL(yuv2rgb_lds_kernel, dim3(cus < a.h ? cus : a.h), dim3(1024), lds, s, a);
        return hipGetLastError();
    }
    hipLaunchKernelGGL(yuv2rgb_kernel, image_grid(a.w, a.h), dim3(256), 0, s, a);
    return hipGetLastError();
}
hipError_t launch_mad(const float *bands, size_t n, int nsub, int *histo, float *out, hipStream_t s)
{
    int *scr = histo + (size_t)nsub * 65536;
    hipError_t e = hipMemsetAsync(histo, 0, ((size_t)nsub * 65536 + (size_t)nsub * MAD_SCRATCH_INTS_PER_BAND) * sizeof(int), s);
    if (e != hipSuccess) return e;
    hipLaunchKernelGGL(mad_sample_kernel, dim3(64, nsub), dim3(256), 0, s, bands, n, scr);
    hipLaunchKernelGGL(mad_pick_kernel, dim3(nsub), dim3(256), 0, s, scr);
    hipLaunchKernelGGL(mad_window_kernel, dim3(flat_grid((long long)n, MAD_GRID), nsub), dim3(256), 0, s, bands, n, scr);
    hipLaunchKernelGGL(mad_window_finish_kernel, dim3(nsub), dim3(64), 0, s, scr, (int)n, out);
    hipLaunchKernelGGL(mad_hist_kernel, dim3(flat_grid((long long)n, MAD_GRID), nsub), dim3(256), 0, s, bands, n, histo, (const int *)scr);
    hipLaunchKernelGGL(mad_finish_kernel, dim3(nsub), dim3(256), 0, s, (const int *)histo, (int)n, out, (const int *)scr);
    return hipGetLastError();
}
hipError_t launch_shrink_sf(const ShrinkArgs &a, int nsub, bool ab, hipStream_t s)
{
    dim3 grid(flat_grid((long long)a.n, 1024), nsub);
    if (ab) hipLaunchKernelGGL(shrink_sf_AB_kernel, grid, dim3(256), 0, s, a);
    else hipLaunchKernelGGL(shrink_sf_L_kernel, grid, dim3(256), 0, s, a);
    return hipGetLastError();
}
hipError_t launch_bishrink_AB(const ShrinkArgs &a, int nsub, hipStream_t s)
{
    hipLaunchKernelGGL(bishrink_AB_kernel, dim3(flat_grid((long long)a.n, 1024), nsub), dim3(256), 0, s, a);
    return hipGetLastError();
}
hipError_t launch_hblur(const BlurArgs &a, int nsub, hipStream_t s)
{
    int maxr = 0;
    for (int l = 0; l < 10; ++l) maxr = a.rad[l] > maxr ? a.rad[l] : maxr;
    if (maxr > HBLUR_MAX_RADIUS) return hipErrorInvalidValue;
    if (maxr > 63) {
        const size_t lds = ((size_t)HB_ROWS * (HBB_COLS + 2 * maxr + 3) + (size_t)HB_ROWS * (HBB_COLS + 1)) * sizeof(float);
        hipError_t e = hipFuncSetAttribute(reinterpret_cast<const void *>(hblur_big_kernel), hipFuncAttributeMaxDynamicSharedMemorySize, (int)lds);
        if (e != hipSuccess) return e;
        hipLaunchKernelGGL(hblur_big_kernel, dim3((a.h + HB_ROWS - 1) / HB_ROWS, nsub), dim3(64), lds, s, a);
        return hipGetLastError();
    }
    const dim3 grid((a.h + HB_ROWS - 1) / HB_ROWS, nsub);
    if (maxr <= 15) {
        if (a.steady_div) hipLaunchKernelGGL((hblur_kernel<15, true>), grid, dim3(64), 0, s, a);
        else hipLaunchKernelGGL((hblur_kernel<15, false>), grid, dim3(64), 0, s, a);
    } else {
        if (a.steady_div) hipLaunchKernelGGL((hblur_kernel<63, true>), grid, dim3(64), 0, s, a);
        else hipLaunchKernelGGL((hblur_kernel<63, false>), grid, dim3(64), 0, s, a);
    }
    return hipGetLastError();
}
hipError_t launch_vblur_combine(const BlurArgs &a, int nsub, hipStream_t s)
{
    if (a.plain) hipLaunchKernelGGL(vblur_combine_kernel<true>, dim3((a.w + 63) / 64, nsub), dim3(64), 0, s, a);
    else hipLaunchKernelGGL(vblur_combine_kernel<false>, dim3((a.w + 63) / 64, nsub), dim3(64), 0, s, a);
    return hipGetLastError();
}

__global__ void __launch_bounds__(256) chroma_map_kernel(ChromaMapArgs a)
{
    const float t0 = 1.f + 1.f * (4.f * lutf_lookup<true>(a.curve, 501, 100.f / 60.f));
    const float cn100 = t0 * t0;
    FOR_IMAGE_XY(ii, jj, a.wid, a.hei) {
        const long long t = (long long)ii * a.wid + jj;
        float RL, GL, BL;
        if (a.gi.on) {
            const size_t o = (size_t)(a.gi.sy1 + 2 * ii) * a.gi.stride + a.gi.sx1 + 2 * jj;
            RL = a.gi.src[0][o]; GL = a.gi.src[1][o]; BL = a.gi.src[2][o];
            gi_convert(a.gi, RL, GL, BL);
        } else {
            const size_t o = (size_t)(2 * ii) * a.stride + 2 * jj;
            RL = a.src[0][o]; GL = a.src[1][o]; BL = a.src[2][o];
        }
        if (a.has_mat) {
            const double dr = RL, dg = GL, db = BL;
            RL = (float)(a.mat[0] * dr + a.mat[1] * dg + a.mat[2] * db);
            GL = (float)(a.mat[3] * dr + a.mat[4] * dg + a.mat[5] * db);
            BL = (float)(a.mat[6] * dr + a.mat[7] * dg + a.mat[8] * db);
        }
        const float XL = a.wpi[0] * RL + a.wpi[1] * GL + a.wpi[2] * BL;
        const float YL = a.wpi[3] * RL + a.wpi[4] * GL + a.wpi[5] * BL;
        const float ZL = a.wpi[6] * RL + a.wpi[7] * GL + a.wpi[8] * BL;
        const float fx = xyz2lab_f(a.cachef, XL / 0.9642f), fy = xyz2lab_f(a.cachef, YL), fz = xyz2lab_f(a.cachef, ZL / 0.8249f);
        const float A = 500.0f * (fx - fy), B = 200.0f * (fy - fz);
        const float cN = sqrtf(A * A + B * B);
        float r = cn100;
        if (cN > 100) {
            const float u = 1.f + 1.f * (4.f * lutf_lookup<true>(a.curve, 501, cN / 60.f));
            r = u * u;
        }
        a.out[t] = r;
    }
}
__device__ __forceinline__ float xyz2lab_f_lds(const float *lds, const float *__restrict__ cachef, float f)
{
    if (f != f) return f;
    if (f < 0.f) return (float)(327.68 * (((24389.0 / 27.0) * (double)f / (double)65535.f + 16.0) / 116.0));
    if (f > 65535.f) return 327.68f * xcbrtf_s(f / 65535.f);
    return lutf_lookup_lds<false>(lds, cachef, 65536, f);
}
__global__ void __launch_bounds__(1024) chroma_map_lds_kernel(ChromaMapArgs a)
{
    extern __shared__ float dn_lut_lds[];
    lut_lds_fill(dn_lut_lds, a.cachef, 1024);
    const float t0 = 1.f + 1.f * (4.f * lutf_lookup<true>(a.curve, 501, 100.f / 60.f));
    const float cn100 = t0 * t0;
    constexpr int NR = 2, NPX = 4;
    const float *const p0 = a.gi.on ? a.gi.src[0] : a.src[0], *const p1 = a.gi.on ? a.gi.src[1] : a.src[1], *const p2 = a.gi.on ? a.gi.src[2] : a.src[2];
    for (int yb = blockIdx.x; yb < a.hei; yb += NR * gridDim.x)
        for (int x0 = 0; x0 < a.wid; x0 += NPX * 1024) {
            float r[NR * NPX], g[NR * NPX], b[NR * NPX];
#pragma unroll
            for (int k = 0; k < NR * NPX; ++k) {
                const int jj = x0 + (k % NPX) * 1024 + (int)threadIdx.x, ir = yb + (k / NPX) * (int)gridDim.x, ii = ir < a.hei ? ir : a.hei - 1;
                const int jc = jj < a.wid ? jj : a.wid - 1;
                const size_t o = a.gi.on ? (size_t)(a.gi.sy1 + 2 * ii) * a.gi.stride + a.gi.sx1 + 2 * jc : (size_t)(2 * ii) * a.stride + 2 * jc;
                r[k] = p0[o]; g[k] = p1[o]; b[k] = p2[o];
            }
#pragma unroll
            for (int k = 0; k < NR * NPX; ++k) {
                const int jj = x0 + (k % NPX) * 1024 + (int)threadIdx.x, ii = yb + (k / NPX) * (int)gridDim.x;
                if (jj >= a.wid || ii >= a.hei) continue;
                float RL = r[k], GL = g[k], BL = b[k];
                if (a.gi.on) gi_convert(a.gi, RL, GL, BL);
                if (a.has_mat) {
                    const double dr = RL, dg = GL, db = BL;
                    RL = (float)(a.mat[0] * dr + a.mat[1] * dg + a.mat[2] * db);
                    GL = (float)(a.mat[3] * dr + a.mat[4] * dg + a.mat[5] * db);
                    BL = (float)(a.mat[6] * dr + a.mat[7] * dg + a.mat[8] * db);
                }
                const float XL = a.wpi[0] * RL + a.wpi[1] * GL + a.wpi[2] * BL;
                const float YL = a.wpi[3] * RL + a.wpi[4] * GL + a.wpi[5] * BL;
                const float ZL = a.wpi[6] * RL + a.wpi[7] * GL + a.wpi[8] * BL;
                const float fx = xyz2lab_f_lds(dn_lut_lds, a.cachef, XL / 0.9642f), fy = xyz2lab_f_lds(dn_lut_lds, a.cachef, YL), fz = xyz2lab_f_lds(dn_lut_lds, a.cachef, ZL / 0.8249f);
                const float A = 500.0f * (fx - fy), B = 200.0f * (fy - fz);
                const float cN = sqrtf(A * A + B * B);
                float res = cn100;
                if (cN > 100) {
                    const float u = 1.f + 1.f * (4.f * lutf_lookup<true>(a.curve, 501, cN / 60.f));
                    res = u * u;
                }
                a.out[(long long)ii * a.wid + jj] = res;
            }
        }
}
hipError_t launch_chroma_map(const ChromaMapArgs &a, hipStream_t s)
{
    if ((long long)a.wid * a.hei >= (1 << 20) && (reinterpret_cast<uintptr_t>(a.cachef) & 15) == 0 && !a.no_lds_lut && device_block_fits(LUT_LDS_N * (int)sizeof(float), 1024)) {
        const size_t lds = (size_t)LUT_LDS_N * sizeof(float);
        hipError_t e = dyn_lds_once(reinterpret_cast<const void *>(chroma_map_lds_kernel), (int)lds);
        if (e != hipSuccess) return e;
        int dev = 0, cus = 256;
        if (hipGetDevice(&dev) == hipSuccess) (void)hipDeviceGetAttribute(&cus, hipDeviceAttributeMultiprocessorCount, dev);
        if (a.cu_reserve > 0) cus = cus - a.cu_reserve > 1 ? cus - a.cu_reserve : 1;
        hipLaunchKernelGGL(chroma_map_lds_kernel, dim3(cus < a.hei ? cus : a.hei), dim3(1024), lds, s, a);
        return hipGetLastError();
    }
    hipLaunchKernelGGL(chroma_map_kernel, image_grid(a.wid, a.hei), dim3(256), 0, s, a);
    return hipGetLastError();
}

__device__ __forceinline__ float dninfo_fetch(const DnInfoArgs &a, int c, size_t si)
{
    float t = 0.f;
    t += a.src[c][si];
    t *= a.mul[c];
    if (a.do_clip) t = std_max(0.f, std_min(t, 65535.f));
    return t;
}
__global__ void __launch_bounds__(256) dninfo_maps_kernel(DnInfoArgs a)
// ... 60 lines not shown
```

### art_amd/csrc/kernels.h

```cpp
#pragma once
#include <hip/hip_runtime.h>
#include "paramcurve.h"
#include <vector>
#include <stddef.h>
#include <stdint.h>
#include <mutex>
#include <set>
#include <utility>

inline hipError_t dyn_lds_once(const void *fn, int bytes)
{
    static std::mutex m;
    static std::set<std::pair<const void *, int>> done;
    int dev = 0;
    hipError_t e = hipGetDevice(&dev);
    if (e != hipSuccess) return e;
    std::lock_guard<std::mutex> lk(m);
    if (done.count({fn, dev})) return hipSuccess;
    e = hipFuncSetAttribute(fn, hipFuncAttributeMaxDynamicSharedMemorySize, bytes);
    if (e == hipSuccess) done.insert({fn, dev});
    return e;
}

inline bool device_block_fits(int lds_bytes, int threads)
// ... 138 lines not shown
    double mat[9];
    float exp_scale, black;
    int chain_n;
    float chain_scale[2], chain_black[2];
    const float *lut;
    float whitept;
    int tail_kind;
    double tail_y;
    ParamCurve tail_pc;
    int no_lds_lut;
    int cu_reserve;
};
hipError_t launch_get_image_convert(const PixArgs &a, hipStream_t s);
hipError_t launch_exposure(const PixArgs &a, hipStream_t s);
hipError_t launch_tone_std(const PixArgs &a, hipStream_t s);
hipError_t launch_yuv_mode(const PixArgs &a, hipStream_t s);
struct ScaleArgs {
    const void *src; size_t src_stride;
    int src_u16;
    float *dst; size_t dst_stride;
    int w, h;
    int cfa[36];
    int bayer;
    float cblacksom[4], scale_mul[4];
    int *chmax_bits;
};
hipError_t launch_scale_colors(const ScaleArgs &a, hipStream_t s);
struct DnInfoArgs {
    const float *src[3];
    size_t stride;
    float mul[3];
    int do_clip;
    int sx[9], sy[9];
    int crW, crH, wid, hei;
    double mat[9];
    float wp[9];
    const float *cachef, *cachefy, *gamcurve;
    float gain, gam, gamthresh, gamslope;
    float *maps;
    float *A, *B;
    int crop;
    float *stats;
};
hipError_t launch_dninfo_maps(const DnInfoArgs &a, hipStream_t s);
hipError_t launch_dninfo_stats(const DnInfoArgs &a, hipStream_t s);
hipError_t launch_dninfo_ab(const DnInfoArgs &a, hipStream_t s);
hipError_t launch_ordered_sum(const float *x, long long n, float *out, hipStream_t s);
struct MixArgs { float *dst[3]; size_t stride; int w, h; float m[9]; const float *lut[3]; };
hipError_t launch_channel_mixer(const MixArgs &a, hipStream_t s);
hipError_t launch_rgb_curves(const MixArgs &a, hipStream_t s);
struct HslCurve { const double *x, *y, *slope; int n; };
struct HslArgs {
    float *img[3]; size_t stride; int w, h;
    float ws1[3];
    HslCurve curve[4];
    float *mask;
    int which, to_rgb;
};
hipError_t launch_hsl_prepare(const HslArgs &a, hipStream_t s);
hipError_t launch_hsl_mask(const HslArgs &a, hipStream_t s);
hipError_t launch_hsl_apply(const HslArgs &a, hipStream_t s);
hipError_t launch_hsl_finish(const HslArgs &a, hipStream_t s);
struct LabArgs {
    float *img[3]; size_t stride; int w, h;
    float ws[9], iws[9];
    const float *cachef, *cachefy;
    const float *lcurve, *acurve, *bcurve;
    float chroma;
    unsigned *hist;
};
hipError_t launch_rgb_to_lab(const LabArgs &a, hipStream_t s);
hipError_t launch_lab_to_rgb(const LabArgs &a, hipStream_t s);
hipError_t launch_lab_hist(const LabArgs &a, hipStream_t s);
hipError_t launch_lab_adjust(const LabArgs &a, hipStream_t s);
struct DualArgs {
    float *rgb[3]; size_t stride;
    const float *raw; size_t raw_stride;
    int w, h; unsigned filters;
    const float *cachefy;
    float *L, *blend;
    float threshold;
};
hipError_t launch_rgb2l(const DualArgs &a, hipStream_t s);
hipError_t launch_blend_mask(const DualArgs &a, hipStream_t s);
hipError_t launch_tile_stats(const DualArgs &a, int nH, int nW, int y0, int x0, int step, int ts, float *var, hipStream_t s);
hipError_t launch_contrast_threshold(const DualArgs &a, int ty, int tx, int ts, float *result, hipStream_t s);
hipError_t launch_bilinear_blend(const DualArgs &a, hipStream_t s);
constexpr int VNG4_CODE_INTS = 320;
struct Vng4Args {
    const float *raw; size_t raw_stride;
    float *red, *green, *blue; size_t out_stride;
    float *image;
    const int *code;
    int w, h; unsigned filters, prefilters;
};
unsigned vng4_prefilters(unsigned filters);
void vng4_build_code(unsigned pf, int width, int *codes);
hipError_t launch_vng4(const Vng4Args &a, hipStream_t s);
hipError_t launch_dual_blend_planes(const DualArgs &a, const float *r2, const float *g2, const float *b2, size_t s2, hipStream_t s);
struct LogEncArgs {
    float *img[3]; size_t stride; int w, h;
    double ws1[3];
    float gray, shadows_range, dynamic_range, linbase, blend;
    int satcontrol;
    int hlcompr;
    float hlcompr_factor, compr_p, compr_s;
    float *Y, *Y2;
};
hipError_t launch_logenc_direct(const LogEncArgs &a, hipStream_t s);
hipError_t launch_logenc_prepare(const LogEncArgs &a, hipStream_t s);
hipError_t launch_logenc_blend(const LogEncArgs &a, hipStream_t s);
float logenc_find_gray(float source_gray, float target_gray);
bool flat_curve_polyline(const double *pts, int npts, bool periodic, int ppn, double identity, std::vector<double> &x, std::vector<double> &y, std::vector<double> &slope);
struct OutArgs {
    const float *src[3]; size_t src_stride; float *dst[3]; size_t dst_stride; int w, h;
    float m[9]; int linear; const float *lut; int lutsz; int *unsupported;
    unsigned char *out; size_t out_stride_bytes; int bps, is_float;
};
hipError_t launch_rgb2out_matrix(const OutArgs &a, hipStream_t s);
hipError_t launch_scanlines(const OutArgs &a, hipStream_t s);
bool scanlines_host_ok(const OutArgs &a);
hipError_t launch_scanlines_host(const OutArgs &a, int workgroups, hipStream_t s);
struct SatArgs { float *dst[3]; size_t stride; int w, h; float saturation, vibrance; int vib; double ws1[3]; };
hipError_t launch_saturation_vibrance(const SatArgs &a, hipStream_t s);
struct NeutralArgs {
    float *img[3]; size_t stride; int w, h;
    const float *lut;
    const float *pq, *pq_inv;
    float *hues;
    float ws[9], iws[9], to_out[9], to_work[9];
    float whitecoeff;
    int tail_kind;
    double tail_y;
    ParamCurve tail_pc;
    int no_lds_lut;
    int cu_reserve;
};
hipError_t launch_neutral_hues(const NeutralArgs &a, hipStream_t s);
hipError_t launch_tone_neutral(const NeutralArgs &a, hipStream_t s);
void build_pq_luts(float *pq65536, float *pq_inv65536);
void dninfo_band_stats(const float *mad_a, const float *mad_b, int nbands, bool aggressive, float out[6]);
void dninfo_reduce(const float info[9][16], bool aggressive, float ch_M[9], float max_r[9], float max_b[9], float out3[3]);

struct WaveArgs {
    const float *src;
    size_t src_stride;
    float *lo;
    float *b1, *b2, *b3;
    float *dst;
    size_t dst_stride;
    int w, h, w2, h2;
    int skip;
    float blend;
};
hipError_t launch_wavelet_analysis0(const WaveArgs &a, hipStream_t s);
hipError_t launch_wavelet_haar_analysis(const WaveArgs &a, hipStream_t s);
hipError_t launch_wavelet_haar_synthesis(const WaveArgs &a, hipStream_t s);
hipError_t launch_wavelet_synthesis0(const WaveArgs &a, hipStream_t s);

struct GetImageFuse {
    int on;
    const float *src[3];
    size_t stride;
    int sx1, sy1;
    float mul[3];
    int do_clip, has_mat;
    double mat[9];
};
struct DnPixArgs {
    GetImageFuse gi;
    float exp_scale, exp_black;
    int exp_on;
    float *rgb[3];
    size_t stride;
    float *L, *A, *B;
    int w, h;
    float gain, newGain;
    float gam, gamthresh, gamslope, igam, igamthresh, igamslope;
    const float *gamcurve, *igamcurve;
    float ws1[3];
    float realred, realblue, qhighFactor;
    float pre_scale, post_scale;
    int lab_mode;
    int igam_lds_lo;
    float wpi[9], iws[9];
    const float *cachef, *cachefy, *dn_gamma, *dn_igamma;
    int no_lds_lut;
    int cu_reserve;
};
struct ChromaMapArgs {
    GetImageFuse gi;
    const float *src[3]; size_t stride;
    int wid, hei;
    int has_mat; double mat[9];
    float wpi[9];
    const float *cachef;
    const float *curve;
    float *out;
    int no_lds_lut;
    int cu_reserve;
};
hipError_t launch_chroma_map(const ChromaMapArgs &a, hipStream_t s);
bool flat_curve_sample(const double *pts, int npts, bool periodic, int ppn, double identity, int nout, double *out);
float noise_curve_lut(const double *pts, int npts, float lut[501]);
void build_cachef(float *lut65536);
void build_cachefy(float *lut65536);
void build_denoise_gamma_tabs(float *gtab65536, float *igtab65536);

struct ShrinkArgs {
    float *coef;
    const float *coefL;
    float *sfave;
    size_t n;
    const float *madL;
    const float *madab;
    const float *noisevar;
    float noisevar_const;
    float noisevar_scale;
    float noisevar_ab;
    int useNoiseCCurve;
};
struct BlurArgs {
    const float *src;
    float *dst;
    const float *sfave;
    float *coef;
    size_t n;
    int w, h;
    int rad[10];
    int steady_div;
    int plain;
    int level0;
};
constexpr int HBLUR_MAX_RADIUS = 900;
hipError_t launch_gamma_lut(float *lut, float gamma, float start, float slope, float divisor, float factor, hipStream_t s);
hipError_t launch_rgb2yuv(const DnPixArgs &a, hipStream_t s);
hipError_t launch_yuv2rgb(const DnPixArgs &a, hipStream_t s);
hipError_t launch_bishrink_AB(const ShrinkArgs &a, int nsub, hipStream_t s);
constexpr int MAD_SCRATCH_INTS_PER_BAND = 8 + 1024 + 4096 + 8;
hipError_t launch_mad(const float *bands, size_t n, int nsub, int *histo, float *out, hipStream_t s);
hipError_t launch_shrink_sf(const ShrinkArgs &a, int nsub, bool ab, hipStream_t s);
hipError_t launch_hblur(const BlurArgs &a, int nsub, hipStream_t s);
hipError_t launch_vblur_combine(const BlurArgs &a, int nsub, hipStream_t s);
struct FusedShrinkArgs {
    const float *coef;
    float *coef_out;
    float *coefC;
    const float *coefL;
    size_t n;
    int w, h;
    const float *madL;
    const float *madab;
    const float *noisevar;
    int noisevar_nonneg;
    float noisevar_const;
    float noisevar_scale;
    float noisevar_ab[2];
    int useNoiseCCurve;
    int rad[10];
    int level0;
    int nsub;
    int nL;
    int nsub_ch;
    int mad_ch_stride;
    int nstrips;
    float *hand;
    int wpad;
    int *progress;
    int *ticket;
    int *diag;
    long long wait_ticks;
    int stall_band, stall_strip;
    long long *prof;
};
bool shrink_blur_supported(int w, int h, const int *rad, int level0, int nsub);
size_t shrink_blur_scratch_floats(int w, int h, int nsub, int maxr);
hipError_t launch_shrink_blur(FusedShrinkArgs a, float *scratch, hipStream_t s);

struct DetailArgs {
    float *L;
    const float *Lin;
    const float *tm_in, *tm_out;
    const float *costab, *costab_t;
    float *blocks;
    int w, h, numblox_W, numblox_H;
    float detail_hi, detail_lo;
    int blur_rad;
    const float *mask;
    float params_Ldetail;
    int plain;
    int inside32;
};
hipError_t launch_detail_blocks(const DetailArgs &a, hipStream_t s);
hipError_t launch_detail_gather(const DetailArgs &a, hipStream_t s);

struct GuidedArgs {
    float *rgb[3];
    size_t stride;
    int W, H;
    int w, h;
    float *in[3];
    float *guide;
    float *chan[3];
    float *low[8];
    double ws1[3];
    float epsilon;
    int nch;
    float *q; size_t q_stride;
};
hipError_t launch_gf_prepare(const GuidedArgs &a, hipStream_t s);
hipError_t launch_gf_subsample(const GuidedArgs &a, hipStream_t s);
hipError_t launch_gf_ab(const GuidedArgs &a, hipStream_t s);
hipError_t launch_gf_finish(const GuidedArgs &a, hipStream_t s);
hipError_t launch_gf_finish_plain(const GuidedArgs &a, hipStream_t s);

struct MaskArgs {
    const float *src; size_t src_stride;
    float *L2, *m2;
    float *mask;
    int W, H, w4, h4;
    float scaling, threshold, ceiling, factor;
};
struct GaussArgs {
    float *img, *tmp;
    double *tmp64;
    int W, H;
    double B, b[3], M[9];
    float Bf, bf[3], Mf[9];
};
struct NlmArgs {
    float *img; size_t img_stride;
    float *src;
    float *mask;
    float *SW;
    float *explut;
    int W, H, WW, HH, border, search_radius, patch_radius, ntiles_x, ntiles_y;
    float factor, h2;
};
hipError_t launch_detail_mask(const MaskArgs &a, hipStream_t s);
hipError_t launch_gaussian(const GaussArgs &a, hipStream_t s);
hipError_t launch_gaussian3(float *img, float *tmp, int W, int H, float c0, float c1, hipStream_t s);
hipError_t launch_nlm(const NlmArgs &a, hipStream_t s);
bool nlm_group_supported(const NlmArgs &a);
hipError_t launch_nlm_group(const NlmArgs &a, hipStream_t s);

struct CaArgs {
    float *raw; size_t stride;
    int W, H, width;
    unsigned cfa;
    int vblsz, hblsz, ntv, nth;
    int fw, fh;
    float *Gtmp, *RawDataTmp;
    float *blockwt, *blockshifts;
    float *blockfit;
    float *oldraw, *red, *blue;
    double *fit;
    int *words;
    int autoCA;
    double cared, cablue;
};
hipError_t launch_ca_capture(const CaArgs &a, hipStream_t s);
hipError_t launch_ca_iteration(const CaArgs &a, hipStream_t s);
hipError_t launch_ca_factors(const CaArgs &a, hipStream_t s);
hipError_t launch_ca_apply(const CaArgs &a, hipStream_t s);
hipError_t launch_ca_step(const CaArgs &a, hipStream_t s);

constexpr int LC_CHUNK = 4096;
struct LcSegStats {
    double sum;
    double vari;
    int cnt;
    float maxv, minv;
    float avg;
};
struct LcStatArgs {
    const float *bands;
    const float *coeff0;
    size_t n;
    int nbands, nchunk;
    double *psum; int *pcnt; float *pmax, *pmin;
    LcSegStats *res;
};
struct LcLevelConst { int on; float mean, thr, logmax, rap, asig, bsig, amean; };
struct LcRemapArgs {
    float *bands, *coeff0;
    size_t n;
    int nlevels;
    const float *curve;
    LcLevelConst lv[10];
    int c0_on;
    float ave, ah, bh, al, bl;
};
struct LcBlendArgs {
// ... 15 lines not shown
```

### art_amd/csrc/wavelet.hip

```cpp
#include <hip/hip_runtime.h>
#include "devmath.h"
#include "kernels.h"

namespace artgpu {

namespace {
__constant__ float DAUB_LO[6] = {0.f, 0.f, 0.34150635f, 0.59150635f, 0.15849365f, -0.091506351f};
__constant__ float DAUB_HI[6] = {-0.091506351f, -0.15849365f, 0.59150635f, -0.34150635f, 0.f, 0.f};
__constant__ float SYN_LO[6] = {-0.091506351f, 0.15849365f, 0.59150635f, 0.34150635f, 0.f, 0.f};
__constant__ float SYN_HI[6] = {0.f, 0.f, -0.34150635f, 0.59150635f, -0.15849365f, -0.091506351f};
__device__ __forceinline__ int clampi(int v, int lo, int hi) { return v < lo ? lo : (v > hi ? hi : v); }

#ifndef A0_TW_
#define A0_TW_ 64
#endif
#ifndef A0_TH_
#ifdef A0_PLAIN
#define A0_TH_ 16
#else
#define A0_TH_ 32
#endif
#endif
constexpr int A0_TW = A0_TW_, A0_TH = A0_TH_;
constexpr int A0_LW = 2 * A0_TW + 6;
#ifndef S0_TW_
#define S0_TW_ 128
#endif
#ifndef S0_TH_
#define S0_TH_ 32
#endif
constexpr int S0_TW = S0_TW_, S0_TH = S0_TH_;
constexpr int S0_LH = S0_TH / 2 + 4;
}

#ifdef A0_PLAIN
__global__ void __launch_bounds__(256) wavelet_analysis0_kernel(WaveArgs a)
{
    __shared__ float tLo[A0_TH][A0_LW], tHi[A0_TH][A0_LW];
    const int w = a.w, h = a.h, w2 = a.w2;
    const int c0 = blockIdx.x * A0_TW, r0 = blockIdx.y * A0_TH;
    const int icol0 = 2 * c0 - 3;
    for (int t = threadIdx.x; t < A0_TH * A0_LW; t += 256) {
        const int rr = t / A0_LW, cc = t - rr * A0_LW;
        const int orow = r0 + rr;
        if (orow >= a.h2) continue;
        const int row = 2 * orow;
        const int k = clampi(icol0 + cc, 0, w - 1);
        float l = 0.f, hh = 0.f;
#pragma unroll
        for (int j = 0; j < 6; ++j) {
            const float s = a.src[(size_t)clampi(row + (2 - j), 0, h - 1) * a.src_stride + k];
            l += DAUB_LO[j] * s;
            hh += DAUB_HI[j] * s;
        }
        tLo[rr][cc] = l;
        tHi[rr][cc] = hh;
    }
    __syncthreads();
    for (int t = threadIdx.x; t < A0_TH * A0_TW; t += 256) {
        const int rr = t / A0_TW, cc = t - rr * A0_TW;
        const int orow = r0 + rr, ocol = c0 + cc;
        if (orow >= a.h2 || ocol >= w2) continue;
        const int i = 2 * ocol;
        float l0 = 0.f, h0 = 0.f, l1 = 0.f, h1 = 0.f;
#pragma unroll
        for (int j = 0; j < 6; ++j) {
            const int x = clampi(i + (2 - j), 0, w - 1) - icol0;
            const float sl = tLo[rr][x], sh = tHi[rr][x];
            l0 += DAUB_LO[j] * sl; h0 += DAUB_HI[j] * sl;
            l1 += DAUB_LO[j] * sh; h1 += DAUB_HI[j] * sh;
        }
        const size_t o = (size_t)orow * w2 + ocol;
        a.lo[o] = l0; a.b1[o] = h0; a.b2[o] = l1; a.b3[o] = h1;
    }
}

#else
constexpr int A0_WR = 16;
static_assert(A0_TW == 64 && A0_TH * 128 == 256 * A0_WR, "the walkers' mapping: 128 tmp columns x A0_TH / A0_WR row groups = 256 threads");
__global__ void __launch_bounds__(256) wavelet_analysis0_kernel(WaveArgs a)
{
    __shared__ float tLo[A0_TH][A0_LW], tHi[A0_TH][A0_LW];
    const int w = a.w, h = a.h, w2 = a.w2;
    const int c0 = blockIdx.x * A0_TW, r0 = blockIdx.y * A0_TH;
    const int icol0 = 2 * c0 - 3;
    {
        const int g = threadIdx.x >> 7, cc = threadIdx.x & 127;
        const int orow0 = r0 + g * A0_WR;
        const int k = clampi(icol0 + cc, 0, w - 1);
        const int b0 = 2 * orow0 - 3;
        float v[2 * A0_WR + 4];
#pragma unroll
        for (int i = 0; i < 2 * A0_WR + 4; ++i) v[i] = a.src[(size_t)clampi(b0 + i, 0, h - 1) * a.src_stride + k];
        const int hr = threadIdx.x / 6, hc = 128 + (int)threadIdx.x - hr * 6;
        const bool halo = hr < A0_TH;
        const int hk = clampi(icol0 + hc, 0, w - 1), hrow = 2 * (r0 + (halo ? hr : 0));
        float hv[6];
#pragma unroll
        for (int j = 0; j < 6; ++j) hv[j] = a.src[(size_t)clampi(hrow + (2 - j), 0, h - 1) * a.src_stride + hk];
#pragma unroll
        for (int q = 0; q < A0_WR; ++q) {
            float l = 0.f, hh = 0.f;
#pragma unroll
            for (int j = 0; j < 6; ++j) {
                const float sv = v[2 * q + 5 - j];
                l += DAUB_LO[j] * sv;
                hh += DAUB_HI[j] * sv;
            }
            if (orow0 + q < a.h2) {
                tLo[g * A0_WR + q][cc] = l;
                tHi[g * A0_WR + q][cc] = hh;
            }
        }
        if (halo && r0 + hr < a.h2) {
            float l = 0.f, hh = 0.f;
#pragma unroll
            for (int j = 0; j < 6; ++j) {
                l += DAUB_LO[j] * hv[j];
                hh += DAUB_HI[j] * hv[j];
            }
            tLo[hr][hc] = l;
            tHi[hr][hc] = hh;
        }
    }
    __syncthreads();
    for (int t = threadIdx.x; t < A0_TH * A0_TW; t += 256) {
        const int rr = t / A0_TW, cc = t - rr * A0_TW;
        const int orow = r0 + rr, ocol = c0 + cc;
        if (orow >= a.h2 || ocol >= w2) continue;
        const int i = 2 * ocol;
        float l0 = 0.f, h0 = 0.f, l1 = 0.f, h1 = 0.f;
#pragma unroll
        for (int j = 0; j < 6; ++j) {
            const int x = clampi(i + (2 - j), 0, w - 1) - icol0;
            const float sl = tLo[rr][x], sh = tHi[rr][x];
            l0 += DAUB_LO[j] * sl; h0 += DAUB_HI[j] * sl;
            l1 += DAUB_LO[j] * sh; h1 += DAUB_HI[j] * sh;
        }
        const size_t o = (size_t)orow * w2 + ocol;
        a.lo[o] = l0; a.b1[o] = h0; a.b2[o] = l1; a.b3[o] = h1;
    }
}
#endif

__global__ void __launch_bounds__(256) wavelet_haar_analysis_kernel(WaveArgs a)
{
    const int w = a.w2, h = a.h2, skip = a.skip;
    const long long n = (long long)w * h;
    for (long long t = blockIdx.x * (long long)blockDim.x + threadIdx.x; t < n; t += (long long)gridDim.x * blockDim.x) {
        const int row = (int)(t / w), i = (int)(t - (long long)row * w);
        const int rp = row < h - skip ? row + skip : row - skip;
        const int ip = i < w - skip ? i + skip : i - skip;
        const float s00 = a.src[(size_t)row * w + i], s01 = a.src[(size_t)row * w + ip];
        const float s10 = a.src[(size_t)rp * w + i], s11 = a.src[(size_t)rp * w + ip];
        const float tl0 = 0.25f * (s00 + s10), tl1 = 0.25f * (s01 + s11);
        const float th0 = 0.25f * (s00 - s10), th1 = 0.25f * (s01 - s11);
        a.lo[t] = tl0 + tl1; a.b1[t] = tl0 - tl1;
        a.b2[t] = th0 + th1; a.b3[t] = th0 - th1;
    }
}

__device__ __forceinline__ float haar_syn(float lo, float hi, float lop, float hip, bool first)
{
    return first ? (lo + hi) : 0.5f * (lo + hi + lop - hip);
}
__global__ void __launch_bounds__(256) wavelet_haar_synthesis_kernel(WaveArgs a)
{
    const int w = a.w2, h = a.h2, skip = a.skip;
    const long long n = (long long)w * h;
    for (long long t = blockIdx.x * (long long)blockDim.x + threadIdx.x; t < n; t += (long long)gridDim.x * blockDim.x) {
        const int row = (int)(t / w), j = (int)(t - (long long)row * w);
        const bool fj = j < skip, fr = row < skip;
        const int jp = fj ? j : j - skip, rp = fr ? row : row - skip;
        const size_t o00 = (size_t)row * w + j, o01 = (size_t)row * w + jp, o10 = (size_t)rp * w + j, o11 = (size_t)rp * w + jp;
        const float tLo0 = haar_syn(a.src[o00], a.b1[o00], a.src[o01], a.b1[o01], fj);
        const float tHi0 = haar_syn(a.b2[o00], a.b3[o00], a.b2[o01], a.b3[o01], fj);
        float r;
        if (fr) {
            r = tLo0 + tHi0;
        } else {
            const float tLo1 = haar_syn(a.src[o10], a.b1[o10], a.src[o11], a.b1[o11], fj);
            const float tHi1 = haar_syn(a.b2[o10], a.b3[o10], a.b2[o11], a.b3[o11], fj);
            r = 0.5f * (tLo0 + tHi0 + tLo1 - tHi1);
        }
        a.lo[t] = r;
    }
}

__global__ void __launch_bounds__(256) wavelet_synthesis0_kernel(WaveArgs a)
{
    __shared__ float tLo[S0_LH][S0_TW], tHi[S0_LH][S0_TW];
    const int w = a.w, h = a.h, w2 = a.w2, h2 = a.h2;
    const int c0 = blockIdx.x * S0_TW, r0 = blockIdx.y * S0_TH;
    constexpr int shift = 3;
    const int srow0 = (r0 + shift) / 2 - 2;
    constexpr int NP = S0_TW / 2 + 1;
    constexpr int NI = (S0_LH * NP + 255) / 256, NH = (NI + 1) / 2;
#pragma unroll
    for (int half = 0; half < 2; ++half) {
        float vs[NH][3], v1[NH][3], v2[NH][3], v3[NH][3];
#pragma unroll
        for (int n = 0; n < NH; ++n) {
            const int t = min((int)threadIdx.x + (half * NH + n) * 256, S0_LH * NP - 1);
            const int rr = t / NP, p = t - rr * NP;
            const int i1 = min(c0 + 2 * p - 1, w - 1);
            const int k = clampi(srow0 + rr, 0, h2 - 1);
            const int i_src = (i1 + shift) / 2;
#pragma unroll
            for (int l = 0; l < 3; ++l) {
                const size_t arg = (size_t)k * w2 + clampi(i_src - l, 0, w2 - 1);
                vs[n][l] = a.src[arg]; v1[n][l] = a.b1[arg]; v2[n][l] = a.b2[arg]; v3[n][l] = a.b3[arg];
            }
        }
#pragma unroll
        for (int n = 0; n < NH; ++n) {
            const int t = (int)threadIdx.x + (half * NH + n) * 256;
            if (half * NH + n >= NI || t >= S0_LH * NP) continue;
            const int rr = t / NP, p = t - rr * NP;
            const int cc1 = 2 * p - 1, cc2 = 2 * p;
            const int i1 = c0 + cc1;
            if (i1 >= w) continue;
            float lo1 = 0.f, hi1 = 0.f, lo2 = 0.f, hi2 = 0.f;
#pragma unroll
            for (int l = 0; l < 3; ++l) {
                const float s = vs[n][l], d1 = v1[n][l], d2 = v2[n][l], d3 = v3[n][l];
                lo1 += (SYN_LO[2 * l] * s + SYN_HI[2 * l] * d1);
                hi1 += (SYN_LO[2 * l] * d2 + SYN_HI[2 * l] * d3);
                lo2 += (SYN_LO[2 * l + 1] * s + SYN_HI[2 * l + 1] * d1);
                hi2 += (SYN_LO[2 * l + 1] * d2 + SYN_HI[2 * l + 1] * d3);
            }
            if (cc1 >= 0) { tLo[rr][cc1] = lo1; tHi[rr][cc1] = hi1; }
            if (cc2 < S0_TW && i1 + 1 < w) { tLo[rr][cc2] = lo2; tHi[rr][cc2] = hi2; }
        }
    }
    __syncthreads();
    const float srcFactor = 1.f - a.blend;
    constexpr int NIT = S0_TH * S0_TW / 256;
    static_assert((256 / S0_TW) % 2 == 0 && S0_TH % 2 == 0, "row parity per thread");
    const bool odd_tap = ((r0 + (int)threadIdx.x / S0_TW + shift) & 1) != 0;
    float flo[3], fhi[3];
#pragma unroll
    for (int l = 0; l < 3; ++l) { flo[l] = odd_tap ? SYN_LO[2 * l + 1] : SYN_LO[2 * l]; fhi[l] = odd_tap ? SYN_HI[2 * l + 1] : SYN_HI[2 * l]; }
    float dv[NIT];
    const bool use_old = a.blend != 1.f;
#pragma unroll
    for (int n = 0; n < NIT; ++n) {
        const int t = threadIdx.x + n * 256;
        const int rr = t / S0_TW, cc = t - rr * S0_TW;
        const int i = min(r0 + rr, h - 1), k = min(c0 + cc, w - 1);
        dv[n] = use_old ? a.dst[(size_t)i * a.dst_stride + k] : 0.f;
    }
#pragma unroll
    for (int n = 0; n < NIT; ++n) {
        const int t = threadIdx.x + n * 256;
        const int rr = t / S0_TW, cc = t - rr * S0_TW;
        const int i = r0 + rr, k = c0 + cc;
        if (i >= h || k >= w) continue;
        const int i_src = (i + shift) / 2;
        float tot = 0.f;
#pragma unroll
        for (int l = 0; l < 3; ++l) {
            const int lr = clampi(i_src - l, 0, h2 - 1) - srow0;
            tot += (flo[l] * tLo[lr][cc] + fhi[l] * tHi[lr][cc]);
        }
        const size_t o = (size_t)i * a.dst_stride + k;
        a.dst[o] = dv[n] * srcFactor + a.blend * 4.f * tot;
    }
}

hipError_t launch_wavelet_analysis0(const WaveArgs &a, hipStream_t s)
{
    dim3 grid((a.w2 + A0_TW - 1) / A0_TW, (a.h2 + A0_TH - 1) / A0_TH);
    hipLaunchKernelGGL(wavelet_analysis0_kernel, grid, dim3(256), 0, s, a);
    return hipGetLastError();
}
static int flat_grid(long long n) { long long g = (n + 255) / 256; return (int)(g < 16384 ? g : 16384); }
hipError_t launch_wavelet_haar_analysis(const WaveArgs &a, hipStream_t s)
{
    hipLaunchKernelGGL(wavelet_haar_analysis_kernel, dim3(flat_grid((long long)a.w2 * a.h2)), dim3(256), 0, s, a);
    return hipGetLastError();
}
hipError_t launch_wavelet_haar_synthesis(const WaveArgs &a, hipStream_t s)
{
    hipLaunchKernelGGL(wavelet_haar_synthesis_kernel, dim3(flat_grid((long long)a.w2 * a.h2)), dim3(256), 0, s, a);
    return hipGetLastError();
}
hipError_t launch_wavelet_synthesis0(const WaveArgs &a, hipStream_t s)
{
    dim3 grid((a.w + S0_TW - 1) / S0_TW, (a.h + S0_TH - 1) / S0_TH);
    hipLaunchKernelGGL(wavelet_synthesis0_kernel, grid, dim3(256), 0, s, a);
    return hipGetLastError();
}

}
```

Before: 4535 MP/s.

## Fold MAD histogram counting into wavelet analysis kernels

```diff
diff --git a/art_amd/csrc/artgpu_api.hip b/art_amd/csrc/artgpu_api.hip
--- a/art_amd/csrc/artgpu_api.hip
+++ b/art_amd/csrc/artgpu_api.hip
@@ -35,6 +35,8 @@
         int opt_dn_streams = 0;
         int opt_dn_fused = 1;
         int opt_dn_detail_plain = 0;
+        int opt_dn_mad_fold = 1;
+        int opt_dn_mad_fold_grid = 0;
         int opt_dn_debug_stall = -1;
         long opt_dn_wait_ms = 0;
         int opt_io_direct = -1;
@@ -70,6 +72,7 @@
     std::string err;
     int *fs_diag = nullptr;
     long long batch_px = 0;
+    const int *dn_fold_flags = nullptr; int dn_fold_ranges[8][2] = {}; int dn_fold_nranges = 0;
     int dn_form = -1, dn_form_streak = 0;
     float *arena = nullptr;
     size_t arena_bytes = 0;
@@ -456,6 +459,29 @@
         *value = v;
         return ARTGPU_OK;
     }
+    if (n == "dn_mad_fold") { *value = ctx->shared.opt_dn_mad_fold; return ARTGPU_OK; }
+    if (n.rfind("dn_mad_bits", 0) == 0 && n.size() > 11) {
+        const int k = std::atoi(n.c_str() + 11);
+        if (k < 0 || k > 95 || !ctx->dn_fold_flags) return fail(ctx, ARTGPU_EINVAL, "get_option: %s: word 0 .. 95 of a context that has denoised", name);
+        HIPCHK(ctx, hipSetDevice(ctx->device));
+        HIPCHK(ctx, hipStreamSynchronize(ctx->stream));
+        int v = 0;
+        HIPCHK(ctx, hipMemcpy(&v, ctx->dn_fold_flags - 96 + k, sizeof v, hipMemcpyDeviceToHost));
+        *value = v;
+        return ARTGPU_OK;
+    }
+    if (n == "dn_mad_fold_settled" || n == "dn_mad_fold_fallback") {
+        HIPCHK(ctx, hipSetDevice(ctx->device));
+        HIPCHK(ctx, hipStreamSynchronize(ctx->stream));
+        int flags[96] = {};
+        if (ctx->dn_fold_nranges) HIPCHK(ctx, hipMemcpy(flags, ctx->dn_fold_flags, sizeof flags, hipMemcpyDeviceToHost));
+        const int want = n == "dn_mad_fold_settled" ? 1 : 2;
+        long cnt = 0;
+        for (int r = 0; r < ctx->dn_fold_nranges; ++r)
+            for (int k = 0; k < ctx->dn_fold_ranges[r][1]; ++k) cnt += flags[ctx->dn_fold_ranges[r][0] + k] == want;
+        *value = cnt;
+        return ARTGPU_OK;
+    }
     return fail(ctx, ARTGPU_EINVAL, "get_option: unknown option '%s'", name);
 }
 
@@ -473,6 +499,8 @@
     else if (n == "roctx") ctx->shared.opt_roctx = value != 0;
     else if (n == "dn_streams") ctx->shared.opt_dn_streams = value != 0;
     else if (n == "dn_fused") ctx->shared.opt_dn_fused = (int)value;
+    else if (n == "dn_mad_fold") ctx->shared.opt_dn_mad_fold = value != 0;
+    else if (n == "dn_mad_fold_grid") { if (value < 0 || value > 65536) return fail(ctx, ARTGPU_EINVAL, "dn_mad_fold_grid: 0 (default) .. 65536 workgroups"); ctx->shared.opt_dn_mad_fold_grid = (int)value; }
     else if (n == "dn_detail_plain") { if (value < 0 || value > 3) return fail(ctx, ARTGPU_EINVAL, "dn_detail_plain: 0 .. 3"); ctx->shared.opt_dn_detail_plain = (int)value; }
     else if (n == "dn_debug_stall") ctx->shared.opt_dn_debug_stall = (int)value;
     else if (n == "dn_wait_ms") ctx->shared.opt_dn_wait_ms = value < 0 ? 0 : value;
@@ -533,6 +561,7 @@
     for (int k = 0; k < artgpu_ctx::NPOOL; ++k) drop(&ctx->pool[k], &ctx->pool_bytes[k]);
     ctx->batch_px = 0;
     ctx->gam_tab = nullptr;
+    ctx->dn_fold_flags = nullptr; ctx->dn_fold_nranges = 0;
     ctx->ncurve_host.clear();
     for (int k = 0; k < 3; ++k) ctx->rgbcurve_host[k].clear();
     int rc = ARTGPU_OK;
@@ -1063,6 +1092,7 @@
        P_MK_WORK, P_MK_TAB, P_MK_CTHR, P_MK_AREA, P_MK_OUT,
        P_CC_MASK, P_CC_OOR, P_CC_GEN,
        P_SM_PLANES, P_SM_MASK, P_SM_BOX, P_SM_GEN,
+       P_MADPART,
        P_NSLOTS };
 static_assert(P_NSLOTS <= artgpu_ctx::NPOOL, "grow artgpu_ctx::pool");
 
@@ -1070,6 +1100,8 @@
     float *bands, *low[2];
     int cur, nlevels, w, h, w2, h2;
     size_t n;
+    int *cnt;
+    int g0, g1;
     float *band(int l, int dir) const { return bands + ((size_t)l * 3 + (dir - 1)) * n; }
 };
 
@@ -1078,14 +1110,18 @@
     if (!st) st = ctx->stream;
     WaveArgs a = {};
     a.w = d.w; a.h = d.h; a.w2 = d.w2; a.h2 = d.h2;
+    if (d.cnt) HIPCHK(ctx, hipMemsetAsync(d.cnt, 0, (size_t)3 * d.nlevels * MAD_FOLD_NB * sizeof(int), st));
     for (int l = 0; l < d.nlevels; ++l) {
+        a.cnt = d.cnt ? d.cnt + (size_t)l * 3 * MAD_FOLD_NB : nullptr;
         a.b1 = d.band(l, 1); a.b2 = d.band(l, 2); a.b3 = d.band(l, 3);
         if (l == 0) {
             a.src = src; a.src_stride = src_stride ? src_stride : (size_t)d.w; a.lo = d.low[0]; d.cur = 0;
-            HIPCHK(ctx, launch_wavelet_analysis0(a, st));
+            a.cnt_grid = d.g0;
+            HIPCHK(ctx, d.cnt ? launch_wavelet_analysis0_count(a, st) : launch_wavelet_analysis0(a, st));
         } else {
             a.src = d.low[d.cur]; a.lo = d.low[d.cur ^ 1]; a.skip = wavelet_skip(l);
-            HIPCHK(ctx, launch_wavelet_haar_analysis(a, st));
+            a.cnt_grid = d.g1;
+            HIPCHK(ctx, d.cnt ? launch_wavelet_haar_analysis_count(a, st) : launch_wavelet_haar_analysis(a, st));
             d.cur ^= 1;
         }
     }
@@ -1217,6 +1253,8 @@
     bool too_small;
     int rad[10], maxrad;
     bool fork;
+    bool mad_fold;
+    int fold_g0, fold_g1;
     bool fused, merged, merged_mad;
     bool two_chroma;
     int detail_plain;
@@ -1225,7 +1263,7 @@
 };
 
 DnPlan dn_plan(int w, int h, const artgpu_denoise_params *p, double scale, double expcomp, uint32_t flags, bool want_resid, bool has_ccalc,
-               int opt_dn_streams, int opt_dn_fused, int opt_dn_detail_plain, long opt_dn_wait_ms, int opt_dn_debug_stall)
+               int opt_dn_streams, int opt_dn_fused, int opt_dn_detail_plain, long opt_dn_wait_ms, int opt_dn_debug_stall, int opt_dn_mad_fold, int opt_dn_mad_fold_grid)
 {
     DnPlan pl = {};
     const int w2 = (w + 1) / 2, h2 = (h + 1) / 2;
@@ -1289,6 +1327,8 @@
                 (autoch || (noisevarab_r > 0.001f && noisevarab_b > 0.001f));
     pl.merged_mad = pl.merged && opt_dn_fused != 3;
     pl.two_chroma = pl.fork || pl.merged;
+    pl.fold_g0 = mad_fold_grid_a0(w2, h2, opt_dn_mad_fold_grid); pl.fold_g1 = mad_fold_grid_haar(pl.n2, opt_dn_mad_fold_grid);
+    pl.mad_fold = opt_dn_mad_fold != 0 && mad_fold_a0_fits(w2, h2, pl.fold_g0) && mad_fold_haar_fits(pl.n2, pl.fold_g1);
     return pl;
 }
 
@@ -1297,6 +1337,8 @@
     float *sfc[3], *tmpc[3], *histo_fc[3];
     DevDecomp Ld, Cdd[2];
     float *fused_scratch, *Lbands2;
+    int *fold_cnt;
+    int *fold_flags;
 };
 
 int pool_drop(artgpu_ctx *ctx, int slot)
@@ -1326,8 +1368,14 @@
         (rc = pool_get(ctx, P_LBANDS, (merged_mad ? 3 : 1) * band_bytes, &Ld.bands)) || (rc = pool_get(ctx, P_LLOW0, n2 * 4, &Ld.low[0])) || (rc = pool_get(ctx, P_LLOW1, n2 * 4, &Ld.low[1])) ||
         (rc = merged_mad ? ARTGPU_OK : pool_get(ctx, P_CBANDS, (merged ? 2 : 1) * band_bytes, &Cdd[0].bands)) || (rc = pool_get(ctx, P_CLOW0, n2 * 4, &Cdd[0].low[0])) || (rc = pool_get(ctx, P_CLOW1, n2 * 4, &Cdd[0].low[1])) ||
         (rc = pool_get(ctx, P_HISTO, (merged_mad ? 3 : 1) * histo_bytes, &b.histo_fc[0])) ||
-        (rc = pool_get(ctx, P_MAD, 3 * 32 * 4, &b.mad)) || (rc = pool_get(ctx, P_GAM, 2 * 65536 * 4, &b.gamlut)))
+        (rc = pool_get(ctx, P_MAD, 2 * 3 * 32 * 4, &b.mad)) || (rc = pool_get(ctx, P_GAM, 2 * 65536 * 4, &b.gamlut)))
         return rc;
+    b.fold_flags = reinterpret_cast<int *>(b.mad) + 96;
+    if (pl.mad_fold) {
+        float *pf;
+        if ((rc = pool_get(ctx, P_MADPART, (size_t)(merged_mad ? 3 : 1) * nsub * MAD_FOLD_NB * sizeof(int), &pf))) return rc;
+        b.fold_cnt = reinterpret_cast<int *>(pf);
+    }
     if (ctx->dn_form == (fused ? 1 : 0)) ++ctx->dn_form_streak; else { ctx->dn_form = fused ? 1 : 0; ctx->dn_form_streak = 1; }
     const bool settle = ctx->dn_form_streak >= 4;
     if (fused) {
@@ -1353,6 +1401,12 @@
         b.histo_fc[1] = b.histo_fc[2] = b.histo_fc[0];
         Cdd[1] = Cdd[0];
     }
+    if (pl.mad_fold)
+        for (int c = 0; c < 3; ++c) {
+            DevDecomp &d = c == 0 ? Ld : Cdd[c - 1];
+            d.g0 = pl.fold_g0; d.g1 = pl.fold_g1;
+            d.cnt = b.fold_cnt + (merged_mad ? (size_t)c * nsub * MAD_FOLD_NB : 0);
+        }
     if (pl.useNoiseCCurve) {
         if (!plane_ok(ccalc) || ccalc->w != w2 || ccalc->h != h2) return fail(ctx, ARTGPU_EINVAL, "rgb_denoise: ccalc must be %dx%d", w2, h2);
         if (ccalc->on_device && (size_t)ccalc->row_stride_bytes == (size_t)w2 * 4) {
@@ -1397,6 +1451,14 @@
         return fa;
     }
     int fused_pass(bool ab, const float *cin, float *cout, const float *cL, const float *mL, const float *mab, int lev0, int nb, float nv_const, float noisevar_ab);
+    int mad_decomposed(const float *bands, int nb, int *histo, float *out)
+    {
+        if (!pl.mad_fold) { HIPCHK(ctx, launch_mad(bands, pl.n2, nb, histo, out, sL)); return ARTGPU_OK; }
+        int *flags = b.fold_flags + (out - b.mad);
+        HIPCHK(ctx, launch_mad_fold(bands, pl.n2, nb, pl.nsub, b.fold_cnt, histo, out, flags, sL));
+        if (ctx->dn_fold_nranges < 8) { ctx->dn_fold_ranges[ctx->dn_fold_nranges][0] = (int)(out - b.mad); ctx->dn_fold_ranges[ctx->dn_fold_nranges][1] = nb; ++ctx->dn_fold_nranges; }
+        return ARTGPU_OK;
+    }
     int chroma_front(int ch);
     int chroma_back(int ch);
     int luma(hipStream_t sd);
@@ -1432,7 +1494,7 @@
     int rc2;
     if ((rc2 = decompose_dev(ctx, Cd, ch == 0 ? b.A : b.B, sL))) return rc2;
     if (pl.aggressive && noisevar_ab > 0.001f) {
-        HIPCHK(ctx, launch_mad(Cd.bands, n2, nsub, histo, madab, sL));
+        if ((rc2 = mad_decomposed(Cd.bands, nsub, histo, madab))) return rc2;
         ShrinkArgs sa = {};
         sa.n = n2; sa.noisevar = b.ccalc_dev; sa.noisevar_scale = pl.maxNoiseVarab; sa.noisevar_ab = noisevar_ab; sa.useNoiseCCurve = pl.useNoiseCCurve ? 1 : 0;
         const size_t top = (size_t)(nsub - 3) * n2;
@@ -1454,7 +1516,9 @@
         }
     }
     if (noisevar_ab > 0.001f && !pl.merged_mad) {
-        HIPCHK(ctx, launch_mad(Cd.bands, n2, nsub, histo, ch == 1 && pl.merged ? b.mad + 32 + nsub : madab, sL));
+        float *out = ch == 1 && pl.merged ? b.mad + 32 + nsub : madab;
+        if (pl.aggressive) HIPCHK(ctx, launch_mad(Cd.bands, n2, nsub, histo, out, sL));
+        else if ((rc2 = mad_decomposed(Cd.bands, nsub, histo, out))) return rc2;
         if (!pl.fused) {
             ShrinkArgs sa = {};
             sa.coef = Cd.bands; sa.coefL = Ld.bands; sa.sfave = sf; sa.n = n2; sa.madL = madL; sa.madab = madab;
@@ -1606,7 +1670,7 @@
     if (w > 32767 || h > 32767) return fail(ctx, ARTGPU_EUNSUPPORTED, "rgb_denoise: the reference holds the size in short (FTblockDN.cc:1779)");
     if (p->luminance == 0 && p->chrominance == 0 && !ccalc) return ARTGPU_OK;
     const DnPlan pl = dn_plan(w, h, p, scale, expcomp, flags, nresi || highresi, ccalc != nullptr,
-                              ctx->shared.opt_dn_streams, ctx->shared.opt_dn_fused, ctx->shared.opt_dn_detail_plain, ctx->shared.opt_dn_wait_ms, ctx->shared.opt_dn_debug_stall);
+                              ctx->shared.opt_dn_streams, ctx->shared.opt_dn_fused, ctx->shared.opt_dn_detail_plain, ctx->shared.opt_dn_wait_ms, ctx->shared.opt_dn_debug_stall, ctx->shared.opt_dn_mad_fold, ctx->shared.opt_dn_mad_fold_grid);
     if (pl.too_small) return fail(ctx, ARTGPU_EUNSUPPORTED, "rgb_denoise: %dx%d too small for %d wavelet levels on the device path", w, h, pl.levwav);
     DnBuffers b;
     int rc = dn_buffers(ctx, pl, ccalc, &b);
@@ -1647,13 +1711,14 @@
     px.realred = pl.realred; px.realblue = pl.realblue; px.qhighFactor = pl.aggressive ? 1.f / static_cast<float>(0.9) : 1.0f;
     HIPCHK(ctx, launch_rgb2yuv(px, sL));
 
+    ctx->dn_fold_nranges = 0; ctx->dn_fold_flags = b.fold_flags;
     if ((rc = decompose_dev(ctx, b.Ld, b.L, sL))) return rc;
-    if (!pl.merged_mad) HIPCHK(ctx, launch_mad(b.Ld.bands, pl.n2, pl.nsub, reinterpret_cast<int *>(b.histo_fc[0]), b.mad, sL));
-
     DnRun run = {ctx, pl, b, fu, p, scale, nresi, highresi, sL, {0.f, 0.f}, 0.f, 0.f, b.L};
+    if (!pl.merged_mad && (rc = run.mad_decomposed(b.Ld.bands, pl.nsub, reinterpret_cast<int *>(b.histo_fc[0]), b.mad))) return rc;
+
     if (pl.merged) {
         if ((rc = run.chroma_front(0)) || (rc = run.chroma_front(1))) return rc;
-        if (pl.merged_mad) HIPCHK(ctx, launch_mad(b.Ld.bands, pl.n2, 3 * pl.nsub, reinterpret_cast<int *>(b.histo_fc[0]), b.mad, sL));
+        if (pl.merged_mad && (rc = run.mad_decomposed(b.Ld.bands, 3 * pl.nsub, reinterpret_cast<int *>(b.histo_fc[0]), b.mad))) return rc;
         if ((rc = run.merged_pass())) return rc;
         SideStreamJoin dn_join;
         if (pl.fork) dn_join.arm(ctx->dn_stream[0]);
diff --git a/art_amd/csrc/denoise.hip b/art_amd/csrc/denoise.hip
--- a/art_amd/csrc/denoise.hip
+++ b/art_amd/csrc/denoise.hip
@@ -415,6 +415,35 @@
         }
         out[sub] = r * r;
     }
+}
+
+__global__ void __launch_bounds__(256) mad_count_finish_kernel(const int *cnt, int nsub_ch, int *scr, int datalen, float *out, int *flags)
+{
+    __shared__ int part[256];
+    const int band = blockIdx.x;
+    const int nb = band % nsub_ch < 3 ? MAD_FOLD_NB0 : MAD_FOLD_NB, per = nb / 256;
+    const int *h = cnt + (size_t)band * MAD_FOLD_NB;
+    int *s = scr + (size_t)band * MAD_WIN_STRIDE;
+    int p = 0;
+    for (int i = 0; i < per; ++i) p += h[threadIdx.x * per + i];
+    part[threadIdx.x] = p;
+    __syncthreads();
+    if (threadIdx.x) return;
+    if (datalen <= 1) { out[band] = 0.f; s[0] = 1; if (flags) flags[band] = 1; return; }
+    const int half = datalen / 2;
+    long long total = 0;
+    for (int i = 0; i < 256; ++i) total += part[i];
+    if (total < half) { if (flags) flags[band] = 2; return; }
+    int count = 0, chunk = 0;
+    while (chunk < 256 && count + part[chunk] < half) { count += part[chunk]; ++chunk; }
+    int median = chunk * per;
+    while (count < half) { count += h[median]; ++median; }
+    const int count_ = count - h[median - 1];
+    const float q = ((median - 1) + (half - count_) / ((float)(count - count_)));
+    const float r = (float)((double)q / 0.6745);
+    out[band] = r * r;
+    s[0] = 1;
+    if (flags) flags[band] = 1;
 }
 
 __global__ void __launch_bounds__(256) shrink_sf_L_kernel(ShrinkArgs a)
@@ -849,6 +878,16 @@
     hipLaunchKernelGGL(mad_finish_kernel, dim3(nsub), dim3(256), 0, s, (const int *)histo, (int)n, out, (const int *)scr);
     return hipGetLastError();
 }
+hipError_t launch_mad_fold(const float *bands, size_t n, int nsub, int nsub_ch, const int *cnt, int *histo, float *out, int *flags, hipStream_t s)
+{
+    int *scr = histo + (size_t)nsub * 65536;
+    hipError_t e = hipMemsetAsync(histo, 0, ((size_t)nsub * 65536 + (size_t)nsub * MAD_SCRATCH_INTS_PER_BAND) * sizeof(int), s);
+    if (e != hipSuccess) return e;
+    hipLaunchKernelGGL(mad_count_finish_kernel, dim3(nsub), dim3(256), 0, s, cnt, nsub_ch, scr, (int)n, out, flags);
+    hipLaunchKernelGGL(mad_hist_kernel, dim3(flat_grid((long long)n, MAD_GRID), nsub), dim3(256), 0, s, bands, n, histo, (const int *)scr);
+    hipLaunchKernelGGL(mad_finish_kernel, dim3(nsub), dim3(256), 0, s, (const int *)histo, (int)n, out, (const int *)scr);
+    return hipGetLastError();
+}
 hipError_t launch_shrink_sf(const ShrinkArgs &a, int nsub, bool ab, hipStream_t s)
 {
     dim3 grid(flat_grid((long long)a.n, 1024), nsub);
diff --git a/art_amd/csrc/kernels.h b/art_amd/csrc/kernels.h
--- a/art_amd/csrc/kernels.h
+++ b/art_amd/csrc/kernels.h
@@ -314,9 +314,44 @@
     int w, h, w2, h2;
     int skip;
     float blend;
+    int *cnt;
+    int cnt_grid;
 };
 hipError_t launch_wavelet_analysis0(const WaveArgs &a, hipStream_t s);
 hipError_t launch_wavelet_haar_analysis(const WaveArgs &a, hipStream_t s);
+constexpr int MAD_FOLD_NB = 4096, MAD_FOLD_NB0 = 1024;
+constexpr int MAD_FOLD_A0_TILE_W = 64, MAD_FOLD_A0_TILE_H = 32, MAD_FOLD_HAAR_THREADS = 1024;
+#ifndef MAD_FOLD_A0_GRID
+#define MAD_FOLD_A0_GRID 768
+#endif
+#ifndef MAD_FOLD_HAAR_GRID
+#define MAD_FOLD_HAAR_GRID 512
+#endif
+inline long long mad_fold_a0_tiles(int w2, int h2)
+{
+    return (long long)((w2 + MAD_FOLD_A0_TILE_W - 1) / MAD_FOLD_A0_TILE_W) * ((h2 + MAD_FOLD_A0_TILE_H - 1) / MAD_FOLD_A0_TILE_H);
+}
+inline int mad_fold_grid_a0(int w2, int h2, int cap)
+{
+    const long long t = mad_fold_a0_tiles(w2, h2), c = cap > 0 ? cap : MAD_FOLD_A0_GRID;
+    return (int)(t < c ? t : c);
+}
+inline int mad_fold_grid_haar(size_t n2, int cap)
+{
+    const size_t g = (n2 + MAD_FOLD_HAAR_THREADS - 1) / MAD_FOLD_HAAR_THREADS, c = cap > 0 ? cap : MAD_FOLD_HAAR_GRID;
+    return (int)(g < c ? g : c);
+}
+inline bool mad_fold_a0_fits(int w2, int h2, int g0)
+{
+    return g0 > 0 && (mad_fold_a0_tiles(w2, h2) + g0 - 1) / g0 * (MAD_FOLD_A0_TILE_W * MAD_FOLD_A0_TILE_H / 256) <= 255;
+}
+inline bool mad_fold_haar_fits(size_t n2, int g1)
+{
+    const size_t per = (size_t)g1 * MAD_FOLD_HAAR_THREADS;
+    return g1 > 0 && n2 <= 0x7fffffff && (n2 + per - 1) / per <= 255;
+}
+hipError_t launch_wavelet_analysis0_count(const WaveArgs &a, hipStream_t s);
+hipError_t launch_wavelet_haar_analysis_count(const WaveArgs &a, hipStream_t s);
 hipError_t launch_wavelet_haar_synthesis(const WaveArgs &a, hipStream_t s);
 hipError_t launch_wavelet_synthesis0(const WaveArgs &a, hipStream_t s);
 
@@ -401,6 +436,7 @@
 hipError_t launch_bishrink_AB(const ShrinkArgs &a, int nsub, hipStream_t s);
 constexpr int MAD_SCRATCH_INTS_PER_BAND = 8 + 1024 + 4096 + 8;
 hipError_t launch_mad(const float *bands, size_t n, int nsub, int *histo, float *out, hipStream_t s);
+hipError_t launch_mad_fold(const float *bands, size_t n, int nsub, int nsub_ch, const int *cnt, int *histo, float *out, int *flags, hipStream_t s);
 hipError_t launch_shrink_sf(const ShrinkArgs &a, int nsub, bool ab, hipStream_t s);
 hipError_t launch_hblur(const BlurArgs &a, int nsub, hipStream_t s);
 hipError_t launch_vblur_combine(const BlurArgs &a, int nsub, hipStream_t s);
diff --git a/art_amd/csrc/wavelet.hip b/art_amd/csrc/wavelet.hip
--- a/art_amd/csrc/wavelet.hip
+++ b/art_amd/csrc/wavelet.hip
@@ -31,6 +31,42 @@
 #endif
 constexpr int S0_TW = S0_TW_, S0_TH = S0_TH_;
 constexpr int S0_LH = S0_TH / 2 + 4;
+
+template <int NB>
+__device__ __forceinline__ void mad_count_add(unsigned long long &packed, int *h, float x, bool valid)
+{
+    int v = (int)fminf(fabsf(x), 65535.f);
+    v = valid ? v : 0x10000;
+    packed += (unsigned)v < 8u ? 1ull << (8 * v) : 0ull;
+    if (v >= 8 && v < NB) atomicAdd(&h[v], 1);
+}
+template <int NB>
+__device__ __forceinline__ void mad_count_flush(unsigned long long (&packed)[3], int (*h)[NB])
+{
+#pragma unroll
+    for (int b = 0; b < 3; ++b) {
+        unsigned long long e = packed[b] & 0x00ff00ff00ff00ffull, o = (packed[b] >> 8) & 0x00ff00ff00ff00ffull;
+#pragma unroll
+        for (int s = 32; s > 0; s >>= 1) { e += __shfl_down(e, s); o += __shfl_down(o, s); }
+        if ((threadIdx.x & 63) == 0) {
+#pragma unroll
+            for (int k = 0; k < 4; ++k) {
+                const int ce = (int)((e >> (16 * k)) & 0xffffull), co = (int)((o >> (16 * k)) & 0xffffull);
+                if (ce) atomicAdd(&h[b][2 * k], ce);
+                if (co) atomicAdd(&h[b][2 * k + 1], co);
+            }
+        }
+        packed[b] = 0ull;
+    }
+}
+template <int NB, int THREADS>
+__device__ __forceinline__ void mad_count_store(const WaveArgs &a, const int (*h)[NB])
+{
+    for (int i = threadIdx.x; i < 3 * NB; i += THREADS) {
+        const int b = i / NB, j = i - b * NB, v = h[b][j];
+        if (v) atomicAdd(&a.cnt[b * MAD_FOLD_NB + j], v);
+    }
+}
 }
 
 #ifdef A0_PLAIN
@@ -78,11 +114,12 @@
 #else
 constexpr int A0_WR = 16;
 static_assert(A0_TW == 64 && A0_TH * 128 == 256 * A0_WR, "the walkers' mapping: 128 tmp columns x A0_TH / A0_WR row groups = 256 threads");
-__global__ void __launch_bounds__(256) wavelet_analysis0_kernel(WaveArgs a)
-{
-    __shared__ float tLo[A0_TH][A0_LW], tHi[A0_TH][A0_LW];
+template <bool COUNT>
+__device__ __forceinline__ void analysis0_tile(const WaveArgs &a, int bx, int by, float (*tLo)[A0_LW], float (*tHi)[A0_LW],
+                                               unsigned long long (&packed)[3], int (*hc)[MAD_FOLD_NB0])
+{
     const int w = a.w, h = a.h, w2 = a.w2;
-    const int c0 = blockIdx.x * A0_TW, r0 = blockIdx.y * A0_TH;
+    const int c0 = bx * A0_TW, r0 = by * A0_TH;
     const int icol0 = 2 * c0 - 3;
     {
         const int g = threadIdx.x >> 7, cc = threadIdx.x & 127;
@@ -139,25 +176,95 @@
         }
         const size_t o = (size_t)orow * w2 + ocol;
         a.lo[o] = l0; a.b1[o] = h0; a.b2[o] = l1; a.b3[o] = h1;
-    }
-}
-#endif
-
+        if constexpr (COUNT) {
+            mad_count_add<MAD_FOLD_NB0>(packed[0], hc[0], h0, true);
+            mad_count_add<MAD_FOLD_NB0>(packed[1], hc[1], l1, true);
+            mad_count_add<MAD_FOLD_NB0>(packed[2], hc[2], h1, true);
+        }
+    }
+}
+__global__ void __launch_bounds__(256) wavelet_analysis0_kernel(WaveArgs a)
+{
+    __shared__ float tLo[A0_TH][A0_LW], tHi[A0_TH][A0_LW];
+    unsigned long long none[3];
+    analysis0_tile<false>(a, blockIdx.x, blockIdx.y, tLo, tHi, none, nullptr);
+}
+static_assert(A0_TW == MAD_FOLD_A0_TILE_W && A0_TH == MAD_FOLD_A0_TILE_H, "mad_fold_grid_a0 counts these tiles");
+__global__ void __launch_bounds__(256) wavelet_analysis0_count_kernel(WaveArgs a)
+{
+    __shared__ float tLo[A0_TH][A0_LW], tHi[A0_TH][A0_LW];
+    __shared__ int hc[3][MAD_FOLD_NB0];
+    for (int i = threadIdx.x; i < 3 * MAD_FOLD_NB0; i += 256) (&hc[0][0])[i] = 0;
+    __syncthreads();
+    const int tx = (a.w2 + A0_TW - 1) / A0_TW, ntiles = tx * ((a.h2 + A0_TH - 1) / A0_TH);
+    unsigned long long packed[3] = {0ull, 0ull, 0ull};
+    for (int tile = blockIdx.x; tile < ntiles; tile += gridDim.x) {
+        analysis0_tile<true>(a, tile % tx, tile / tx, tLo, tHi, packed, hc);
+        __syncthreads();
+    }
+    mad_count_flush(packed, hc);
+    __syncthreads();
+    mad_count_store<MAD_FOLD_NB0, 256>(a, hc);
+}
+#endif
+
+__device__ __forceinline__ void haar_analysis_load(const WaveArgs &a, int w, int h, int skip, long long t, float (&s)[4])
+{
+    const int row = (int)(t / w), i = (int)(t - (long long)row * w);
+    const int rp = row < h - skip ? row + skip : row - skip;
+    const int ip = i < w - skip ? i + skip : i - skip;
+    s[0] = a.src[(size_t)row * w + i]; s[1] = a.src[(size_t)row * w + ip];
+    s[2] = a.src[(size_t)rp * w + i]; s[3] = a.src[(size_t)rp * w + ip];
+}
+__device__ __forceinline__ void haar_analysis_sums(const float (&s)[4], float &lo, float &c1, float &c2, float &c3)
+{
+    const float s00 = s[0], s01 = s[1], s10 = s[2], s11 = s[3];
+    const float tl0 = 0.25f * (s00 + s10), tl1 = 0.25f * (s01 + s11);
+    const float th0 = 0.25f * (s00 - s10), th1 = 0.25f * (s01 - s11);
+    lo = tl0 + tl1; c1 = tl0 - tl1; c2 = th0 + th1; c3 = th0 - th1;
+}
+__device__ __forceinline__ void haar_analysis_store(const WaveArgs &a, long long t, float lo, float c1, float c2, float c3)
+{
+    a.lo[t] = lo; a.b1[t] = c1;
+    a.b2[t] = c2; a.b3[t] = c3;
+}
 __global__ void __launch_bounds__(256) wavelet_haar_analysis_kernel(WaveArgs a)
 {
     const int w = a.w2, h = a.h2, skip = a.skip;
     const long long n = (long long)w * h;
     for (long long t = blockIdx.x * (long long)blockDim.x + threadIdx.x; t < n; t += (long long)gridDim.x * blockDim.x) {
-        const int row = (int)(t / w), i = (int)(t - (long long)row * w);
-        const int rp = row < h - skip ? row + skip : row - skip;
-        const int ip = i < w - skip ? i + skip : i - skip;
-        const float s00 = a.src[(size_t)row * w + i], s01 = a.src[(size_t)row * w + ip];
-        const float s10 = a.src[(size_t)rp * w + i], s11 = a.src[(size_t)rp * w + ip];
-        const float tl0 = 0.25f * (s00 + s10), tl1 = 0.25f * (s01 + s11);
-        const float th0 = 0.25f * (s00 - s10), th1 = 0.25f * (s01 - s11);
-        a.lo[t] = tl0 + tl1; a.b1[t] = tl0 - tl1;
-        a.b2[t] = th0 + th1; a.b3[t] = th0 - th1;
-    }
+        float s[4], lo, c1, c2, c3;
+        haar_analysis_load(a, w, h, skip, t, s);
+        haar_analysis_sums(s, lo, c1, c2, c3);
+        haar_analysis_store(a, t, lo, c1, c2, c3);
+    }
+}
+__global__ void __launch_bounds__(MAD_FOLD_HAAR_THREADS) wavelet_haar_analysis_count_kernel(WaveArgs a)
+{
+    constexpr int T = MAD_FOLD_HAAR_THREADS;
+    __shared__ int hc[3][MAD_FOLD_NB];
+    for (int i = threadIdx.x; i < 3 * MAD_FOLD_NB; i += T) (&hc[0][0])[i] = 0;
+    __syncthreads();
+    const int w = a.w2, h = a.h2, skip = a.skip;
+    const long long n = (long long)w * h;
+    unsigned long long packed[3] = {0ull, 0ull, 0ull};
+    for (long long base = blockIdx.x * (long long)T; base < n; base += (long long)gridDim.x * T) {
+        const long long t = base + threadIdx.x;
+        const bool valid = t < n;
+        float c1 = 0.f, c2 = 0.f, c3 = 0.f;
+        if (valid) {
+            float s[4], lo;
+            haar_analysis_load(a, w, h, skip, t, s);
+            haar_analysis_sums(s, lo, c1, c2, c3);
+            haar_analysis_store(a, t, lo, c1, c2, c3);
+        }
+        mad_count_add<MAD_FOLD_NB>(packed[0], hc[0], c1, valid);
+        mad_count_add<MAD_FOLD_NB>(packed[1], hc[1], c2, valid);
+        mad_count_add<MAD_FOLD_NB>(packed[2], hc[2], c3, valid);
+    }
+    mad_count_flush(packed, hc);
+    __syncthreads();
+    mad_count_store<MAD_FOLD_NB, T>(a, hc);
 }
 
 __device__ __forceinline__ float haar_syn(float lo, float hi, float lop, float hip, bool first)
@@ -280,6 +387,22 @@
     hipLaunchKernelGGL(wavelet_haar_analysis_kernel, dim3(flat_grid((long long)a.w2 * a.h2)), dim3(256), 0, s, a);
     return hipGetLastError();
 }
+hipError_t launch_wavelet_analysis0_count(const WaveArgs &a, hipStream_t s)
+{
+#ifdef A0_PLAIN
+    return hipErrorNotSupported;
+#else
+    if (!a.cnt || a.cnt_grid > mad_fold_a0_tiles(a.w2, a.h2) || !mad_fold_a0_fits(a.w2, a.h2, a.cnt_grid)) return hipErrorInvalidValue;
+    hipLaunchKernelGGL(wavelet_analysis0_count_kernel, dim3(a.cnt_grid), dim3(256), 0, s, a);
+    return hipGetLastError();
+#endif
+}
+hipError_t launch_wavelet_haar_analysis_count(const WaveArgs &a, hipStream_t s)
+{
+    if (!a.cnt || !mad_fold_haar_fits((size_t)a.w2 * a.h2, a.cnt_grid)) return hipErrorInvalidValue;
+    hipLaunchKernelGGL(wavelet_haar_analysis_count_kernel, dim3(a.cnt_grid), dim3(MAD_FOLD_HAAR_THREADS), 0, s, a);
+    return hipGetLastError();
+}
 hipError_t launch_wavelet_haar_synthesis(const WaveArgs &a, hipStream_t s)
 {
     hipLaunchKernelGGL(wavelet_haar_synthesis_kernel, dim3(flat_grid((long long)a.w2 * a.h2)), dim3(256), 0, s, a);
```

Measured after the change: 4599 MP/s (median of 6 runs). +1.4%, better.
